# ArturKKK/graphcast-lite

Measured on AMD Instinct MI355X. Metric: training samples/sec (6h windows) + achieved HBM GB/s on mesh GCNConv, higher is better.
Workload: dtype f32

## Files before the change

graphcast-lite_amd/csrc/linear.hip:

```cpp
#include "common.h"
#include "mfma_io.h"
#include "x3.h"

namespace {

using namespace gcl::mfma_io;

#include "gemm_tile.h"

#define gcl_lin_sync() ((abl & 8) != 0)

constexpr int lin_min_waves(int NS, int KT) { return (NS <= 2 && KT <= 64) ? 3 : (NS <= 2 && KT <= 128) ? 2 : 1; }
constexpr bool lin_zpre(int NS, int EPI) { return EPI == 1 && NS >= 4; }

template <int NS, int EPI, int KT, bool VEC>
__global__ __launch_bounds__(256, lin_min_waves(NS, KT)) void linear_mfma_kernel(const float* __restrict__ X, int64_t ldx,
                                                          const float* __restrict__ in_slope,
                                                          const float* __restrict__ W, int32_t ldw, int32_t trans,
                                                          const float* __restrict__ bias, float* __restrict__ Y,
                                                          int64_t ldy, int64_t rows, int32_t K, int32_t N,
                                                          const float* __restrict__ Z, int64_t ldz,
                                                          const float* __restrict__ z_slope,
                                                          double* __restrict__ slope_part, int32_t akind,
                                                          int32_t abl) {
  extern __shared__ __align__(16) float smem[];
  const int KE = (K + 3) & ~3;
  const int KP = KE + 2;
  float* Wl = smem;
  float* Xl = smem + (size_t)NS * 32 * KP;
  const int tid = threadIdx.x, lane = tid & 63, wave = tid >> 6;
  const int NT = blockDim.x;
  const int TM = (NT >> 6) * 32;

  for (int base = 0; base < NS * 32 * KE; base += NT * 8) {
    float wv[8];
#pragma unroll
    for (int u = 0; u < 8; ++u) {
      const int idx = base + u * NT + tid;
      const int j = idx / KE, k = idx - j * KE;
      const bool ok = (idx < NS * 32 * KE) && (j < N) && (k < K);
      const float* src = ok ? (trans ? W + (int64_t)k * ldw + j : W + (int64_t)j * ldw + k)
                            : reinterpret_cast<const float*>(zero4);
      wv[u] = *src;
    }
#pragma unroll
    for (int u = 0; u < 8; ++u) {
      const int idx = base + u * NT + tid;
      const int j = idx / KE, k = idx - j * KE;
      if (idx < NS * 32 * KE) Wl[j * KP + k] = wv[u];
    }
  }
  const float slope = in_slope ? *in_slope : 1.f;
  const bool act = EPI == EPI_BIAS && akind != gcl::kActNone;
  const bool silu = akind == gcl::kActSilu;
  float* Xw = Xl + (size_t)wave * 32 * KP;
  const int64_t ntiles = (rows + TM - 1) / TM;
  double slope_acc = 0.0;
  const float zs = (EPI == EPI_DX && z_slope) ? *z_slope : 1.f;

  constexpr int CPR = VEC ? KT / 4 : KT;
  constexpr int RPI = CPR >= 64 ? 1 : 64 / CPR;
  constexpr int IPR = CPR >= 64 ? CPR / 64 : 1;
  constexpr int NIT = (32 / RPI) * IPR;
  const int rsub = (CPR >= 64) ? 0 : lane / CPR;
  const int csub = (CPR >= 64) ? lane : lane % CPR;
  float pre[VEC ? NIT * 4 : NIT];
  const int64_t rows_ld = (abl & 4) ? 0 : rows;
  auto issue = [&](int64_t tile) {
    const int64_t r0 = tile * TM + wave * 32;
#pragma unroll
    for (int it = 0; it < NIT; ++it) {
      const int64_t row = r0 + (it / IPR) * RPI + rsub;
      const int c = csub + 64 * (it % IPR);
      if (VEC) {
        const bool ok = (c * 4 < K) && (row < rows_ld);
        const float4* p = ok ? reinterpret_cast<const float4*>(X + row * ldx + c * 4) : zero4;
        const float4 v = *p;
        pre[4 * it] = v.x; pre[4 * it + 1] = v.y; pre[4 * it + 2] = v.z; pre[4 * it + 3] = v.w;
      } else {
        const bool ok = (c < K) && (row < rows_ld);
        const float* p = ok ? X + row * ldx + c : reinterpret_cast<const float*>(zero4);
        pre[it] = *p;
      }
    }
  };
  const float pa = (act && !silu) ? slope : 1.f;
  auto commit = [&]() {
    if (act && silu) {
#pragma unroll
      for (int q = 0; q < (VEC ? NIT * 4 : NIT); ++q) pre[q] = gcl::silu_f(pre[q]);
    } else {
#pragma unroll
      for (int q = 0; q < (VEC ? NIT * 4 : NIT); ++q) pre[q] = pre[q] > 0.f ? pre[q] : pre[q] * pa;
    }
#pragma unroll
    for (int it = 0; it < NIT; ++it) {
      const int r = (it / IPR) * RPI + rsub;
      const int c = csub + 64 * (it % IPR);
      if (VEC) {
        if (c * 4 < KE) {
          float2* d = reinterpret_cast<float2*>(Xw + r * KP + c * 4);
          d[0] = make_float2(pre[4 * it], pre[4 * it + 1]);
          d[1] = make_float2(pre[4 * it + 2], pre[4 * it + 3]);
        }
      } else {
        if (c < KE) Xw[r * KP + c] = pre[it];
      }
    }
  };

  float bj[NS];
#pragma unroll
  for (int s = 0; s < NS; ++s) {
    const int j = s * 32 + (lane & 31);
    bj[s] = (EPI == EPI_BIAS && bias && j < N) ? bias[j] : 0.f;
  }
  const bool has_z = (EPI == EPI_DX) && (Z != nullptr);

  issue(blockIdx.x);
  __syncthreads();
  for (int64_t t = blockIdx.x; t < ntiles; t += gridDim.x) {
    if (!gcl_lin_sync()) __builtin_amdgcn_fence(__ATOMIC_ACQ_REL, "wavefront");
    else __syncthreads();
    commit();
    if (gcl_lin_sync()) __syncthreads();
    issue(t + gridDim.x);

    const int64_t r0 = t * TM;
    const int64_t nr = (rows - r0) < TM ? (rows - r0) : TM;
    const __amdgpu_buffer_rsrc_t ry = make_rsrc(Y + r0 * ldy, (abl & 1) ? 0 : win_bytes(nr, ldy, N));
    const __amdgpu_buffer_rsrc_t rz = make_rsrc(has_z ? Z + r0 * ldz : Y, has_z ? win_bytes(nr, ldz, N) : 0);

    f32x16 acc[NS];
#pragma unroll
    for (int s = 0; s < NS; ++s)
#pragma unroll
      for (int r = 0; r < 16; ++r) acc[s][r] = 0.f;

    constexpr bool ZPRE = lin_zpre(NS, EPI);
    float zpre[ZPRE ? NS : 1][16];
    if (ZPRE) {
#pragma unroll
      for (int s = 0; s < NS; ++s) {
        const int j = s * 32 + (lane & 31);
#pragma unroll
        for (int r = 0; r < 16; ++r) {
          const int rr = wave * 32 + d_row(r, lane);
          zpre[ZPRE ? s : 0][r] = buf_ld1(rz, (j < N) ? (unsigned)((rr * ldz + j) * 4) : kOOB);
        }
      }
    }

    const float* ap = Xw + (lane & 31) * KP + 2 * (lane >> 5);
    const float* bp = Wl + (lane & 31) * KP + 2 * (lane >> 5);
    const int nq = (abl & 2) ? 0 : (KE >> 2);
    float2 a_c = *reinterpret_cast<const float2*>(ap);
    float2 b_c[NS];
#pragma unroll
    for (int s = 0; s < NS; ++s) b_c[s] = *reinterpret_cast<const float2*>(bp + s * 32 * KP);
    for (int q = 0; q < nq; ++q) {
      const int qn = (q + 1 < nq) ? q + 1 : q;
      const float2 a_n = *reinterpret_cast<const float2*>(ap + qn * 4);
      float2 b_n[NS];
#pragma unroll
      for (int s = 0; s < NS; ++s) b_n[s] = *reinterpret_cast<const float2*>(bp + s * 32 * KP + qn * 4);
#pragma unroll
      for (int s = 0; s < NS; ++s) acc[s] = __builtin_amdgcn_mfma_f32_32x32x2f32(a_c.x, b_c[s].x, acc[s], 0, 0, 0);
#pragma unroll
      for (int s = 0; s < NS; ++s) acc[s] = __builtin_amdgcn_mfma_f32_32x32x2f32(a_c.y, b_c[s].y, acc[s], 0, 0, 0);
      a_c = a_n;
#pragma unroll
      for (int s = 0; s < NS; ++s) b_c[s] = b_n[s];
    }

#pragma unroll
    for (int s = 0; s < NS; ++s) {
      const int j = s * 32 + (lane & 31);
      const bool jok = j < N;
      if (EPI == EPI_DX) {
        float zv[16];
#pragma unroll
        for (int r = 0; r < 16; ++r) {
          const int rr = wave * 32 + d_row(r, lane);
          if (ZPRE) zv[r] = zpre[ZPRE ? s : 0][r];
          else zv[r] = buf_ld1(rz, jok ? (unsigned)((rr * ldz + j) * 4) : kOOB);
        }
#pragma unroll
        for (int r = 0; r < 16; ++r) {
          const int rr = wave * 32 + d_row(r, lane);
          float v = acc[s][r];
          if (silu) {
            v *= has_z ? gcl::dsilu_f(zv[r]) : 1.f;
          } else {
            const bool neg = has_z && !(zv[r] > 0.f);
            slope_acc += neg ? (double)(v * zv[r]) : 0.0;
            v = neg ? v * zs : v;
          }
          buf_st1<GCL_ST_AUX>(ry, jok ? (unsigned)((rr * ldy + j) * 4) : kOOB, v);
        }
      } else {
#pragma unroll
        for (int r = 0; r < 16; ++r) {
          const int rr = wave * 32 + d_row(r, lane);
          buf_st1<GCL_ST_AUX>(ry, jok ? (unsigned)((rr * ldy + j) * 4) : kOOB, acc[s][r] + bj[s]);
        }
      }
    }
  }

  if (EPI == EPI_DX && slope_part) {
    for (int off = 32; off > 0; off >>= 1) slope_acc += __shfl_down(slope_acc, off, 64);
    __syncthreads();
    double* dred = reinterpret_cast<double*>(smem);
    if (lane == 0) dred[wave] = slope_acc;
    __syncthreads();
    if (tid == 0) {
      double tot = 0.0;
      for (int wv = 0; wv < (NT >> 6); ++wv) tot += dred[wv];
      slope_part[blockIdx.x] = tot;
    }
  }
}

template <int EPI>
__global__ __launch_bounds__(256) void linear_valu_kernel(const float* __restrict__ X, int64_t ldx,
                                                          const float* __restrict__ in_slope,
                                                          const float* __restrict__ W, int32_t ldw, int32_t trans,
                                                          const float* __restrict__ bias, float* __restrict__ Y,
                                                          int64_t ldy, int64_t rows, int32_t K, int32_t N,
                                                          const float* __restrict__ Z, int64_t ldz,
                                                          const float* __restrict__ z_slope,
                                                          double* __restrict__ slope_part, int32_t akind) {
  __shared__ double red[4];
  const float slope = in_slope ? *in_slope : 1.f;
  const bool act = EPI == EPI_BIAS && akind != gcl::kActNone;
  const float zs = (EPI == EPI_DX && z_slope) ? *z_slope : 1.f;
  double slope_acc = 0.0;
  const int64_t total = rows * N;
  for (int64_t idx = (int64_t)blockIdx.x * 256 + threadIdx.x; idx < total; idx += (int64_t)gridDim.x * 256) {
    const int64_t r = idx / N;
    const int j = (int)(idx - r * N);
    float acc = 0.f;
    for (int k = 0; k < K; ++k) {
      float xv = X[r * ldx + k];
      if (act) xv = gcl::act_f(xv, slope, akind);
      const float wv = trans ? W[(int64_t)k * ldw + j] : W[(int64_t)j * ldw + k];
      acc = fmaf(xv, wv, acc);
    }
    if (EPI == EPI_BIAS) {
      if (bias) acc += bias[j];
    } else if (Z) {
      const float z = Z[r * ldz + j];
      if (akind == gcl::kActSilu) {
        acc *= gcl::dsilu_f(z);
      } else if (!(z > 0.f)) {
        slope_acc += (double)(acc * z);
        acc *= zs;
      }
    }
    Y[r * ldy + j] = acc;
  }
  if (EPI == EPI_DX && slope_part) {
    for (int off = 32; off > 0; off >>= 1) slope_acc += __shfl_down(slope_acc, off, 64);
    if ((threadIdx.x & 63) == 0) red[threadIdx.x >> 6] = slope_acc;
    __syncthreads();
    if (threadIdx.x == 0) slope_part[blockIdx.x] = red[0] + red[1] + red[2] + red[3];
  }
}

constexpr int kDwRT = 64;

template <int NO, int NC>
struct DwCfg {
  static constexpr int WO = NO >= 4 ? 4 : NO;
  static constexpr int WC = 4 / WO;
  static constexpr int TO = NO / WO;
  static constexpr int TC = (NC + WC - 1) / WC;
  static constexpr int PRE = 2 * (NO + NC);
  static constexpr int FoutP = NO * 32, FinP = NC * 32;
  static constexpr int min_waves = (PRE <= 8 && TO * TC <= 2) ? 3 : (PRE <= 16 && TO * TC <= 4) ? 2 : 1;
};

template <int NO, int NC, bool VEC>
__global__ __launch_bounds__(256, (DwCfg<NO, NC>::min_waves)) void dw_mfma_kernel(
    const float* __restrict__ dY, int64_t lddy, const float* __restrict__ X, int64_t ldx,
    const float* __restrict__ in_slope, float* __restrict__ part, float* __restrict__ dbpart, int64_t rows,
    int32_t Fin_all, int32_t Fout, int64_t rows_per_block, int32_t akind, int64_t tile_stride) {
  using Cfg = DwCfg<NO, NC>;
  const int ct = blockIdx.y;
  X += (int64_t)ct * 128;
  part += (int64_t)ct * tile_stride;
  if (ct != 0) dbpart = nullptr;
  const int Fin = (Fin_all - ct * 128) < 128 ? (Fin_all - ct * 128) : 128;
  constexpr int WO = Cfg::WO, WC = Cfg::WC, TO = Cfg::TO, TC = Cfg::TC, PRE = Cfg::PRE;
  constexpr int FoutP = Cfg::FoutP, FinP = Cfg::FinP;
  extern __shared__ __align__(16) float smem[];
  float* Yl = smem;
  float* Xl = smem + (size_t)kDwRT * FoutP;
  const int tid = threadIdx.x, lane = tid & 63, wave = tid >> 6;
  const int li = lane & 31, lk = lane >> 5;
  const int wo = wave % WO, wc = wave / WO;
  const float slope = in_slope ? *in_slope : 1.f;
  const bool act = akind != gcl::kActNone;
  const int64_t rb = (int64_t)blockIdx.x * rows_per_block;
  const int64_t re = min(rows, rb + rows_per_block);
  const int nrows = (int)(re - rb);

  f32x16 acc[TO][TC];
#pragma unroll
  for (int a = 0; a < TO; ++a)
#pragma unroll
    for (int c = 0; c < TC; ++c)
#pragma unroll
      for (int r = 0; r < 16; ++r) acc[a][c][r] = 0.f;
  float dbacc[TO];
#pragma unroll
  for (int a = 0; a < TO; ++a) dbacc[a] = 0.f;

  const int rs = tid >> 3, cg = tid & 7;
  float4 pre[PRE];
  const float* ybase = dY + rb * lddy;
  const float* xbase = X + rb * ldx;
  auto ld_slot = [&](const float* base, int rr, int c4, int64_t ld, int F) -> float4 {
    const bool ok = rr < nrows;
    const float* z = reinterpret_cast<const float*>(zero4);
    const float* src = base + (int64_t)rr * ld + c4;
    if (VEC) return *reinterpret_cast<const float4*>((ok && c4 < F) ? src : z);
    float4 v;
    v.x = *((ok && c4 < F) ? src : z);
    v.y = *((ok && c4 + 1 < F) ? src + 1 : z);
    v.z = *((ok && c4 + 2 < F) ? src + 2 : z);
    v.w = *((ok && c4 + 3 < F) ? src + 3 : z);
    return v;
  };
  auto issue = [&](int rel0) {
#pragma unroll
    for (int it = 0; it < PRE; ++it) {
      const int j = it >> 1;
      const int rr = rel0 + rs + 32 * (it & 1);
      if (j < NO) pre[it] = ld_slot(ybase, rr, (cg + 8 * j) * 4, lddy, Fout);
      else pre[it] = ld_slot(xbase, rr, (cg + 8 * (j - NO)) * 4, ldx, Fin);
    }
  };
  auto commit = [&]() {
#pragma unroll
    for (int it = 0; it < PRE; ++it) {
      const int j = it >> 1;
      const int r = rs + 32 * (it & 1);
      float4 v = pre[it];
      if (j < NO) {
        *reinterpret_cast<float4*>(Yl + r * FoutP + (cg + 8 * j) * 4) = v;
      } else {
        if (act) {
          v.x = gcl::act_f(v.x, slope, akind); v.y = gcl::act_f(v.y, slope, akind);
          v.z = gcl::act_f(v.z, slope, akind); v.w = gcl::act_f(v.w, slope, akind);
        }
        *reinterpret_cast<float4*>(Xl + r * FinP + (cg + 8 * (j - NO)) * 4) = v;
      }
    }
  };

  issue(0);
  for (int rel0 = 0; rel0 < nrows; rel0 += kDwRT) {
    __syncthreads();
    commit();
    __syncthreads();
    issue(rel0 + kDwRT);
    const float* yp = Yl + lk * FoutP + li;
    const float* xp = Xl + lk * FinP + li;
    float av[TO], bv[TC];
#pragma unroll
    for (int a = 0; a < TO; ++a) av[a] = yp[(wo + a * WO) * 32];
#pragma unroll
    for (int c = 0; c < TC; ++c) {
      const int sc = wc + c * WC;
      bv[c] = (sc < NC) ? xp[sc * 32] : 0.f;
    }
    for (int k = 0; k < kDwRT; k += 2) {
      const int kn = (k + 2 < kDwRT) ? k + 2 : k;
      float an[TO], bn[TC];
#pragma unroll
      for (int a = 0; a < TO; ++a) an[a] = yp[kn * FoutP + (wo + a * WO) * 32];
#pragma unroll
      for (int c = 0; c < TC; ++c) {
        const int sc = wc + c * WC;
        bn[c] = (sc < NC) ? xp[kn * FinP + sc * 32] : 0.f;
      }
#pragma unroll
      for (int a = 0; a < TO; ++a) {
        dbacc[a] += av[a];
#pragma unroll
        for (int c = 0; c < TC; ++c)
          acc[a][c] = __builtin_amdgcn_mfma_f32_32x32x2f32(av[a], bv[c], acc[a][c], 0, 0, 0);
      }
#pragma unroll
      for (int a = 0; a < TO; ++a) av[a] = an[a];
#pragma unroll
      for (int c = 0; c < TC; ++c) bv[c] = bn[c];
    }
  }

  float* out = part + (size_t)blockIdx.x * FoutP * FinP;
#pragma unroll
  for (int a = 0; a < TO; ++a) {
    const int so = wo + a * WO;
#pragma unroll
    for (int c = 0; c < TC; ++c) {
      const int sc = wc + c * WC;
      if (sc < NC) {
#pragma unroll
        for (int r = 0; r < 16; ++r)
          out[(size_t)(so * 32 + d_row(r, lane)) * FinP + sc * 32 + li] = acc[a][c][r];
      }
    }
    if (dbpart && wc == 0) {
      const float d = dbacc[a] + __shfl_xor(dbacc[a], 32, 64);
      if (lane < 32) dbpart[(size_t)blockIdx.x * FoutP + so * 32 + lane] = d;
    }
  }
}

template <int NO, int NC>
__global__ __launch_bounds__(256, 1) void linear_bwd_fused_kernel(
    const float* __restrict__ dY, int64_t lddy, const float* __restrict__ W, const float* __restrict__ P,
    int64_t ldp, const float* __restrict__ in_slope, float* __restrict__ dX, int64_t lddx, int64_t rows, int32_t Fin,
    int32_t Fout, float* __restrict__ part_dw, float* __restrict__ part_db, float* __restrict__ part_cs,
    double* __restrict__ part_slope) {
  constexpr int FoP = NO * 32, FiP = NC * 32;
  constexpr int KPo = FoP + 2;
  constexpr int TM = 128;
  constexpr int NT = NO * NC;
  constexpr int TPW = (NT + 3) / 4;
  constexpr int CY = FoP / 4;
  constexpr int CP = NC == 3 ? 32 : FiP / 4;
  constexpr int RY = 64 / CY, RP = 64 / CP;
  constexpr int NY = 32 / RY, NP = 32 / RP;
  extern __shared__ __align__(16) float smem[];
  float* Wt = smem;
  float* dYl = Wt + FiP * KPo;
  float* Pl = dYl + TM * KPo;
  const int tid = threadIdx.x, lane = tid & 63, wave = tid >> 6;
  const int li = lane & 31, lk = lane >> 5;

  for (int idx = tid; idx < FiP * FoP; idx += 256) {
    const int c = idx / FoP, o = idx - c * FoP;
    Wt[c * KPo + o] = (c < Fin && o < Fout) ? W[(int64_t)o * Fin + c] : 0.f;
  }
  const bool act = in_slope != nullptr;
  const float slope = act ? *in_slope : 1.f;
  const int64_t ntiles = (rows + TM - 1) / TM;

  f32x16 dw[TPW];
#pragma unroll
  for (int q = 0; q < TPW; ++q)
#pragma unroll
    for (int r = 0; r < 16; ++r) dw[q][r] = 0.f;
  float dbacc[TPW], cs[NC];
#pragma unroll
  for (int q = 0; q < TPW; ++q) dbacc[q] = 0.f;
#pragma unroll
  for (int s2 = 0; s2 < NC; ++s2) cs[s2] = 0.f;
  double slope_acc = 0.0;

  const int ysub = lane / CY, ycol = lane % CY, psub = lane / CP, pcol = lane % CP;
  float4 pre[NY + NP];
  const float4* zero = zero4;
  auto issue = [&](int64_t tile) {
    const int64_t r0 = tile * TM + wave * 32;
#pragma unroll
    for (int it = 0; it < NY; ++it) {
      const int64_t row = r0 + it * RY + ysub;
      const bool ok = (ycol * 4 < Fout) && (row < rows);
      pre[it] = *(ok ? reinterpret_cast<const float4*>(dY + row * lddy + ycol * 4) : zero);
    }
#pragma unroll
    for (int it = 0; it < NP; ++it) {
      const int64_t row = r0 + it * RP + psub;
      const bool ok = (pcol * 4 < Fin) && (row < rows);
      pre[NY + it] = *(ok ? reinterpret_cast<const float4*>(P + row * ldp + pcol * 4) : zero);
    }
  };
  auto commit = [&]() {
#pragma unroll
    for (int it = 0; it < NY; ++it) {
      const int r = wave * 32 + it * RY + ysub;
      float2* d = reinterpret_cast<float2*>(dYl + r * KPo + ycol * 4);
      const float4 v = pre[it];
      d[0] = make_float2(v.x, v.y);
      d[1] = make_float2(v.z, v.w);
    }
#pragma unroll
    for (int it = 0; it < NP; ++it) {
      const int r = wave * 32 + it * RP + psub;
      const float4 v = pre[NY + it];
      if (pcol * 4 < FiP) *reinterpret_cast<float4*>(Pl + r * FiP + pcol * 4) = v;
    }
  };

  issue(blockIdx.x);
  for (int64_t t = blockIdx.x; t < ntiles; t += gridDim.x) {
    __syncthreads();
    commit();
    __syncthreads();
// ... 713 lines not shown
    return gcl::x3_linear_fwd(x, ldx, act, act == GCL_ACT_PRELU ? slope : nullptr, W, bias, y, ldy, rows, Fin, Fout,
                              (hipStream_t)stream);
  if (!addend && ldw == Fin && (use_valu() || panel_fits(Fin, Fout, vec_x, false, (ldw % 4 == 0) && gcl::aligned16(W))))
    return launch_linear<EPI_BIAS>(x, ldx, act == GCL_ACT_PRELU ? slope : nullptr, W, Fin, 0, bias, y, ldy, rows, Fin,
                                   Fout, nullptr, 0, nullptr, nullptr, nullptr, (hipStream_t)stream, act);
  return launch_gemm<EPI_BIAS>(x, ldx, act, act == GCL_ACT_PRELU ? slope : nullptr, W, ldw, 0, bias, y, ldy, rows, Fin,
                               Fout, nullptr, 0, addend, ldadd, nullptr, nullptr, (hipStream_t)stream);
}

extern "C" int gcl_linear_fwd(const float* x, int64_t ldx, const float* in_slope, const float* W, const float* bias,
                              float* y, int64_t ldy, int64_t rows, int32_t Fin, int32_t Fout, gcl_stream_t stream) {
  return gcl_dense_fwd(x, ldx, in_slope ? GCL_ACT_PRELU : GCL_ACT_NONE, in_slope, W, Fin, bias, nullptr, 0, y, ldy, rows,
                       Fin, Fout, stream);
}

static size_t slope_parts_cap(int64_t rows, int32_t Fin) {
  const int64_t g = (int64_t)gt_geom(rows, Fin).grid;
  return (size_t)(g > 4096 ? g : 4096);
}

extern "C" size_t gcl_linear_bwd_ws_bytes(int64_t rows, int32_t Fin, int32_t Fout) {
  size_t nc = (size_t)(Fin + 31) / 32;
  if (nc > 4) nc = 4;
  const size_t FinP = nc * 32;
  size_t no = (size_t)(Fout + 31) / 32;
  no = no <= 2 ? no : no <= 4 ? 4 : 8;
  const size_t FoutP = no * 32;
  const size_t dw = (size_t)kDwBlocks * FoutP * (FinP + 1) * sizeof(float);
  const size_t sl = slope_parts_cap(rows, Fin) * sizeof(double);
  return dw + sl;
}

extern "C" int gcl_dense_bwd_dx(const float* dy, int64_t lddy, const float* W, int64_t ldw, const float* z, int64_t ldz,
                                int32_t act, const float* slope, float* d_slope, const float* addend, int64_t ldadd,
                                float* dx, int64_t lddx, int64_t rows, int32_t Fin, int32_t Fout, void* ws,
                                size_t ws_bytes, gcl_stream_t stream) {
  GCL_CHECK_ARG(dy && W && dx, "dense_bwd_dx: null argument");
  GCL_CHECK_ARG(lddy >= Fout && lddx >= Fin && ldw >= Fin && (!addend || ldadd >= Fin), "dense_bwd_dx: leading dimension too small");
  if (int rc = check_act("dense_bwd_dx", act, slope)) return rc;
  GCL_CHECK_ARG(act == GCL_ACT_NONE || (z && ldz >= Fin), "dense_bwd_dx: activation given without its pre-activation z");
  hipStream_t st = (hipStream_t)stream;
  const float* sl = act == GCL_ACT_PRELU ? slope : nullptr;
  double* slope_part = nullptr;
  if (sl && d_slope) {
    GCL_CHECK_ARG(ws && ws_bytes >= slope_parts_cap(rows, Fin) * sizeof(double) && gcl::aligned16(ws), "dense_bwd_dx: workspace too small");
    slope_part = (double*)ws;
  }
  int nparts = 0, rc;
  const float* zz = act == GCL_ACT_NONE ? nullptr : z;
  const bool vec_x = (Fout % 4 == 0) && (lddy % 4 == 0) && gcl::aligned16(dy);
  if (!addend && ldw == Fin && (use_valu() || panel_fits(Fout, Fin, vec_x, true, (ldw % 4 == 0) && gcl::aligned16(W))))
    rc = launch_linear<EPI_DX>(dy, lddy, nullptr, W, Fin, 1, nullptr, dx, lddx, rows, Fout, Fin, zz, ldz, sl, slope_part,
                               &nparts, st, act);
  else {
    const size_t off = (slope_parts_cap(rows, Fin) * sizeof(double) + 255) & ~(size_t)255;
    const size_t need = off + (size_t)Fin * Fout * sizeof(float);
    if (ws && ws_bytes >= need && gcl::aligned16(ws) && Fout % 4 == 0 && rows >= 4096) {
      float* Wt = reinterpret_cast<float*>(static_cast<char*>(ws) + off);
      hipLaunchKernelGGL(transpose_kernel, dim3((unsigned)gcl::cdiv(Fin, 32), (unsigned)gcl::cdiv(Fout, 32)), dim3(256), 0,
                         st, W, ldw, Wt, Fout, Fin);
      rc = launch_gemm<EPI_DX>(dy, lddy, act, sl, Wt, Fout, 0, nullptr, dx, lddx, rows, Fout, Fin, zz, ldz, addend,
                               ldadd, slope_part, &nparts, st);
    } else {
      rc = launch_gemm<EPI_DX>(dy, lddy, act, sl, W, ldw, 1, nullptr, dx, lddx, rows, Fout, Fin, zz, ldz, addend, ldadd,
                               slope_part, &nparts, st);
    }
  }
  if (rc) return rc;
  if (slope_part && nparts > 0) {
    hipLaunchKernelGGL(reduce_scalar_kernel, dim3(1), dim3(64), 0, st, slope_part, nparts, d_slope);
    GCL_CHECK_LAUNCH();
  }
  return GCL_OK;
}

extern "C" int gcl_linear_bwd_dx(const float* dy, int64_t lddy, const float* W, const float* x, int64_t ldx,
                                 const float* in_slope, float* d_in_slope, float* dx, int64_t lddx, int64_t rows,
                                 int32_t Fin, int32_t Fout, void* ws, size_t ws_bytes, gcl_stream_t stream) {
  GCL_CHECK_ARG(!in_slope || (x && ldx >= Fin), "linear_bwd_dx: in_slope given without the forward input x");
  return gcl_dense_bwd_dx(dy, lddy, W, Fin, in_slope ? x : nullptr, ldx, in_slope ? GCL_ACT_PRELU : GCL_ACT_NONE,
                          in_slope, d_in_slope, nullptr, 0, dx, lddx, rows, Fin, Fout, ws, ws_bytes, stream);
}

static int dw_block(const float* dy, int64_t lddy, const float* x, int64_t ldx, int akind, const float* in_slope,
                    float* dW, int64_t lddw, float* db, int64_t rows, int32_t Fin, int32_t Fout, int32_t accumulate,
                    void* ws, hipStream_t st, gcl_reduce_job* job = nullptr) {
  const int nct = (Fin + 127) / 128;
  const int NC = nct > 1 ? 4 : (Fin + 31) / 32;
  int NO = (Fout + 31) / 32;
  NO = NO <= 2 ? NO : NO <= 4 ? 4 : 8;
  const int FinP = NC * 32, FoutP = NO * 32;
  const size_t lds = (size_t)kDwRT * (FoutP + FinP) * sizeof(float);
  const int64_t cap = (lds > 80 * 1024 ? gcl::kNumCU : kDwBlocks) / nct;
  int64_t nblk = gcl::cdiv(rows, (nct > 1 ? 4 : 2) * kDwRT);
  if (nblk > cap) nblk = cap;
  if (nblk < 1) nblk = 1;
  int64_t rpb = gcl::cdiv(rows, nblk);
  rpb = gcl::cdiv(rpb, kDwRT) * kDwRT;
  nblk = rows > 0 ? gcl::cdiv(rows, rpb) : 1;
  float* part = (float*)ws;
  float* dbpart = part + (size_t)kDwBlocks * FoutP * FinP;
  const int64_t tile_stride = (int64_t)nblk * FoutP * FinP;
  const bool vec = (lddy % 4 == 0) && (ldx % 4 == 0) && gcl::aligned16(dy) && gcl::aligned16(x);
#define GCL_DW3(NO_, NC_, V_)                                                                                     \
  do {                                                                                                            \
    auto kern = dw_mfma_kernel<NO_, NC_, V_>;                                                                     \
    GCL_ENSURE_DYN_LDS(kern, gcl::kLdsBytes);                                                                     \
    hipLaunchKernelGGL(kern, dim3((unsigned)nblk, (unsigned)nct), dim3(256), lds, st, dy, lddy, x, ldx, in_slope, part, \
                       db ? dbpart : nullptr, rows, Fin, Fout, rpb, akind, tile_stride);                          \
  } while (0)
#define GCL_DW2(NO_, NC_)              \
  do {                                 \
    if (vec) GCL_DW3(NO_, NC_, true);  \
    else GCL_DW3(NO_, NC_, false);     \
  } while (0)
#define GCL_DW(NO_)                    \
  do {                                 \
    switch (NC) {                      \
      case 1: GCL_DW2(NO_, 1); break;  \
      case 2: GCL_DW2(NO_, 2); break;  \
      case 3: GCL_DW2(NO_, 3); break;  \
      default: GCL_DW2(NO_, 4); break; \
    }                                  \
  } while (0)
  switch (NO) {
    case 1: GCL_DW(1); break;
    case 2: GCL_DW(2); break;
    case 4: GCL_DW(4); break;
    default: GCL_DW(8); break;
  }
#undef GCL_DW
#undef GCL_DW2
#undef GCL_DW3
  GCL_CHECK_LAUNCH();
  const bool defer = job && nct <= 3 && nblk >= 64 && gcl::aligned16(part) && gcl::aligned16(dbpart) &&
                     tile_stride % 4 == 0 && 2 * tile_stride < ((int64_t)1 << 31);
  if (defer) {
    job[0].part = part;
    job[0].pstride = (int64_t)FoutP * FinP;
    job[0].nparts = (int32_t)nblk;
    for (int c = 0; c < nct; ++c) {
      const int fi = Fin - c * 128 < 128 ? Fin - c * 128 : 128;
      job[0].seg[c].out = dW + c * 128;
      job[0].seg[c].poff = (int32_t)(c * tile_stride);
      job[0].seg[c].count = Fout * FinP;
      job[0].seg[c].pld = FinP;
      job[0].seg[c].cols = fi;
      job[0].seg[c].ldo = (int32_t)lddw;
      job[0].seg[c].acc = accumulate ? 1 : 0;
    }
    if (db) {
      job[1].part = dbpart;
      job[1].pstride = FoutP;
      job[1].nparts = (int32_t)nblk;
      job[1].seg[0].out = db;
      job[1].seg[0].poff = 0;
      job[1].seg[0].count = FoutP;
      job[1].seg[0].pld = FoutP;
      job[1].seg[0].cols = Fout;
      job[1].seg[0].ldo = Fout;
      job[1].seg[0].acc = accumulate ? 1 : 0;
    }
    return GCL_OK;
  }
  for (int ct = 0; ct < nct; ct += 3) {
    RedSeg seg[3] = {{nullptr, 0, 0, 1, 0, 0, 0}, {nullptr, 0, 0, 1, 0, 0, 0}, {nullptr, 0, 0, 1, 0, 0, 0}};
    for (int q = 0; q < 3 && ct + q < nct; ++q) {
      const int c = ct + q;
      const int fi = Fin - c * 128 < 128 ? Fin - c * 128 : 128;
      GCL_CHECK_ARG((int64_t)c * tile_stride < ((int64_t)1 << 31), "dense_bwd_dw: partial workspace offset overflows");
      seg[q] = RedSeg{dW + c * 128, (int32_t)(c * tile_stride), Fout * FinP, FinP, fi, (int32_t)lddw, accumulate};
    }
    launch_reduce_multi(part, (int)nblk, (int64_t)FoutP * FinP, seg[0], seg[1], seg[2], st);
    GCL_CHECK_LAUNCH();
  }
  if (db) return gcl::launch_reduce_parts(dbpart, (int)nblk, (int64_t)FoutP, FoutP, db, Fout, 1, Fout, accumulate, st);
  return GCL_OK;
}

static int dense_bwd_dw_impl(const float* dy, int64_t lddy, const float* x, int64_t ldx, int32_t act,
                             const float* slope, float* dW, int64_t lddw, float* db, int64_t rows, int32_t Fin,
                             int32_t Fout, int32_t accumulate, void* ws, size_t ws_bytes, gcl_stream_t stream,
                             gcl_reduce_job* job) {
  if (job) memset(job, 0, 2 * sizeof(*job));
  if (Fout > 256) job = nullptr;
  GCL_CHECK_ARG(dy && x && dW, "dense_bwd_dw: null argument");
  GCL_CHECK_ARG(lddy >= Fout && ldx >= Fin && lddw >= Fin, "dense_bwd_dw: leading dimension too small");
  GCL_CHECK_ARG(Fin >= 1 && Fout >= 1, "dense_bwd_dw: bad shape");
  GCL_CHECK_ARG(lddw < (1 << 30), "dense_bwd_dw: lddw too large");
  if (int rc = check_act("dense_bwd_dw", act, slope)) return rc;
  GCL_CHECK_ARG(ws && ws_bytes >= gcl_linear_bwd_ws_bytes(rows, Fin, Fout), "dense_bwd_dw: workspace too small");
  const float* sl = act == GCL_ACT_PRELU ? slope : nullptr;
  for (int o0 = 0; o0 < Fout; o0 += 256) {
    const int fo = Fout - o0 < 256 ? Fout - o0 : 256;
    int rc = dw_block(dy + o0, lddy, x, ldx, act, sl, dW + (int64_t)o0 * lddw, lddw, db ? db + o0 : nullptr, rows, Fin,
                      fo, accumulate, ws, (hipStream_t)stream, job);
    if (rc) return rc;
  }
  return GCL_OK;
}

extern "C" int gcl_dense_bwd_dw(const float* dy, int64_t lddy, const float* x, int64_t ldx, int32_t act,
                                const float* slope, float* dW, int64_t lddw, float* db, int64_t rows, int32_t Fin,
                                int32_t Fout, int32_t accumulate, void* ws, size_t ws_bytes, gcl_stream_t stream) {
  return dense_bwd_dw_impl(dy, lddy, x, ldx, act, slope, dW, lddw, db, rows, Fin, Fout, accumulate, ws, ws_bytes, stream,
                           nullptr);
}

extern "C" int gcl_dense_bwd_dw_deferred(const float* dy, int64_t lddy, const float* x, int64_t ldx, int32_t act,
                                         const float* slope, float* dW, int64_t lddw, float* db, int64_t rows,
                                         int32_t Fin, int32_t Fout, int32_t accumulate, void* ws, size_t ws_bytes,
                                         gcl_stream_t stream, gcl_reduce_job* job) {
  GCL_CHECK_ARG(job, "dense_bwd_dw_deferred: null job");
  return dense_bwd_dw_impl(dy, lddy, x, ldx, act, slope, dW, lddw, db, rows, Fin, Fout, accumulate, ws, ws_bytes, stream,
                           job);
}

extern "C" int gcl_linear_bwd_dw_deferred(const float* dy, int64_t lddy, const float* x, int64_t ldx,
                                          const float* in_slope, float* dW, float* db, int64_t rows, int32_t Fin,
                                          int32_t Fout, int32_t accumulate, void* ws, size_t ws_bytes,
                                          gcl_stream_t stream, gcl_reduce_job* job) {
  GCL_CHECK_ARG(job, "linear_bwd_dw_deferred: null job");
  return dense_bwd_dw_impl(dy, lddy, x, ldx, in_slope ? GCL_ACT_PRELU : GCL_ACT_NONE, in_slope, dW, Fin, db, rows, Fin, Fout,
                           accumulate, ws, ws_bytes, stream, job);
}

extern "C" int gcl_linear_bwd_dw(const float* dy, int64_t lddy, const float* x, int64_t ldx, const float* in_slope,
                                 float* dW, float* db, int64_t rows, int32_t Fin, int32_t Fout, int32_t accumulate,
                                 void* ws, size_t ws_bytes, gcl_stream_t stream) {
  return gcl_dense_bwd_dw(dy, lddy, x, ldx, in_slope ? GCL_ACT_PRELU : GCL_ACT_NONE, in_slope, dW, Fin, db, rows, Fin,
                          Fout, accumulate, ws, ws_bytes, stream);
}

static bool fused_ok(const float* dy, int64_t lddy, const float* x, int64_t ldx, const float* dx, int64_t lddx,
                     int32_t Fin, int32_t Fout) {
  const int off = gcl::env_int("GCL_NO_FUSED_BWD", 0) != 0;
  if (off || use_valu()) return false;
  return Fout <= 64 && Fin <= 96 && (lddy >= ((Fout + 3) & ~3)) && (Fin % 4 == 0) && (lddy % 4 == 0) && (ldx % 4 == 0) &&
         (lddx >= Fin) && gcl::aligned16(dy) && gcl::aligned16(x) && dx != nullptr;
}

extern "C" size_t gcl_linear_bwd_all_ws_bytes(int64_t rows, int32_t Fin, int32_t Fout) {
  const size_t FiP = (size_t)((Fin + 31) / 32) * 32, FoP = (size_t)((Fout + 31) / 32) * 32;
  const size_t fused = (size_t)3 * gcl::kNumCU * (FoP * FiP + FoP + FiP) * sizeof(float) + (size_t)3 * gcl::kNumCU * 8 + 64;
  size_t sep = gcl_linear_bwd_ws_bytes(rows, Fin, Fout);
  const size_t cs = gcl_colsum_ws_bytes(rows, Fin);
  if (cs > sep) sep = cs;
  return fused > sep ? fused : sep;
}

static int bwd_all_impl(const float* dy, int64_t lddy, const float* W, const float* x, int64_t ldx,
                        const float* in_slope, float* d_in_slope, float* dx, int64_t lddx, float* dW,
                        float* db, float* colsum_dx, int64_t rows, int32_t Fin, int32_t Fout,
                        int32_t accumulate, void* ws, size_t ws_bytes, gcl_stream_t stream, gcl_reduce_job* job) {
  if (job) memset(job, 0, sizeof(*job));
  GCL_CHECK_ARG(dy && W && x && dx && dW, "linear_bwd_all: null argument");
  GCL_CHECK_ARG(ws && ws_bytes >= gcl_linear_bwd_all_ws_bytes(rows, Fin, Fout), "linear_bwd_all: workspace too small");
  hipStream_t st = (hipStream_t)stream;
  const int acc_dw = (accumulate & GCL_ACC_DW) ? 1 : 0, acc_db = (accumulate & GCL_ACC_DB) ? 1 : 0,
            acc_cs = (accumulate & GCL_ACC_COLSUM) ? 1 : 0;
  if (!fused_ok(dy, lddy, x, ldx, dx, lddx, Fin, Fout) || rows == 0) {
    int rc;
    if (db && acc_db != acc_dw) {
      rc = gcl_linear_bwd_dw(dy, lddy, x, ldx, in_slope, dW, nullptr, rows, Fin, Fout, acc_dw, ws, ws_bytes, stream);
      if (rc) return rc;
      rc = gcl_colsum(dy, lddy, rows, Fout, db, acc_db, ws, ws_bytes, stream);
    } else {
      rc = gcl_linear_bwd_dw(dy, lddy, x, ldx, in_slope, dW, db, rows, Fin, Fout, acc_dw, ws, ws_bytes, stream);
    }
    if (rc) return rc;
    rc = gcl_linear_bwd_dx(dy, lddy, W, in_slope ? x : nullptr, ldx, in_slope, d_in_slope, dx, lddx, rows, Fin, Fout,
                           ws, ws_bytes, stream);
    if (rc) return rc;
    if (colsum_dx) rc = gcl_colsum(dx, lddx, rows, Fin, colsum_dx, acc_cs, ws, ws_bytes, stream);
    return rc;
  }
  const int NO = (Fout + 31) / 32, NC = (Fin + 31) / 32;
  const int FoP = NO * 32, FiP = NC * 32;
  const int no64 = gcl::env_int("GCL_NO_FUSED64", 0) != 0;
  const bool use64 = (NC == 2) && !no64;
  const bool use_x3 = use64 && gcl::x3_linear_bwd_applicable(dy, lddy, x, ldx, dx, lddx, Fin, Fout);
  const int64_t ntiles = gcl::cdiv(rows, use64 ? 64 : 128);
  const int64_t cap = use64 ? 3 * gcl::kNumCU : gcl::kNumCU;
  const int nblk = use_x3 ? gcl::x3_linear_bwd_blocks(rows) : (int)(ntiles < cap ? ntiles : cap);
  const size_t rec_f = (size_t)FoP * FiP + FoP + FiP;
  float* part_dw = (float*)ws;
  float* part_db = part_dw + (size_t)FoP * FiP;
  float* part_cs = part_db + FoP;
  double* part_sl = (double*)(((uintptr_t)(part_dw + (size_t)3 * gcl::kNumCU * rec_f) + 15) & ~(uintptr_t)15);
  const bool want_slope = in_slope && d_in_slope;
  if (use_x3) {
    if (int rc = gcl::x3_linear_bwd(dy, lddy, W, x, ldx, in_slope, dx, lddx, rows, Fin, Fout, part_dw, db ? part_db : nullptr,
                                    colsum_dx ? part_cs : nullptr, want_slope ? part_sl : nullptr, st))
      return rc;
  } else if (use64) {
    const size_t lds64 = ((size_t)FiP * (FoP + 2) + 64 * (size_t)(FoP + 2) + 64 * (size_t)FiP) * sizeof(float);
#define GCL_FB64(NO_)                                                                                             \
  do {                                                                                                            \
    auto kern = linear_bwd_fused64_kernel<NO_>;                                                                   \
    hipLaunchKernelGGL(kern, dim3(nblk), dim3(256), lds64, st, dy, lddy, W, x, ldx, in_slope, dx, lddx, rows, Fin, \
                       Fout, part_dw, db ? part_db : nullptr, colsum_dx ? part_cs : nullptr,                      \
                       want_slope ? part_sl : nullptr);                                                           \
  } while (0)
    if (NO == 1) GCL_FB64(1);
    else GCL_FB64(2);
#undef GCL_FB64
  } else {
  const size_t lds = ((size_t)FiP * (FoP + 2) + 128 * (size_t)(FoP + 2) + 128 * (size_t)FiP) * sizeof(float);
#define GCL_FB(NO_, NC_)                                                                                          \
  do {                                                                                                            \
    auto kern = linear_bwd_fused_kernel<NO_, NC_>;                                                                \
    GCL_ENSURE_DYN_LDS(kern, gcl::kLdsBytes);                                                                     \
    hipLaunchKernelGGL(kern, dim3(nblk), dim3(256), lds, st, dy, lddy, W, x, ldx, in_slope, dx, lddx, rows, Fin,  \
                       Fout, part_dw, db ? part_db : nullptr, colsum_dx ? part_cs : nullptr,                      \
// ... 103 lines not shown
```

graphcast-lite_amd/functional.py:

```python
from typing import List, Optional

import os

import torch

from . import hip


def _grad_slot(p: Optional[torch.Tensor], needs: bool):
    if p is None or not needs:
        return None, False, True
    if p.grad is not None:
        return p.grad, True, True
    return torch.zeros_like(p), False, False


class _Grads:

    def __init__(self, params: List[Optional[torch.Tensor]], needs: List[bool]):
        self.dst, self.acc, self.ret_none = [], [], []
        for p, nd in zip(params, needs):
            d, a, r = _grad_slot(p, nd)
            self.dst.append(d)
            self.acc.append(a)
            self.ret_none.append(r)

    def out(self):
        return tuple(None if r else d for d, r in zip(self.dst, self.ret_none))


_ZERO = {}


def _token(like: torch.Tensor, shape):
    z = _ZERO.get(like.device)
    if z is None:
        if like.is_cuda and torch.cuda.is_current_stream_capturing():
            return like.new_zeros(()).expand(shape)
        with torch.inference_mode(False):
            z = _ZERO[like.device] = torch.zeros((), dtype=torch.float32, device=like.device)
    return z.expand(shape)


_ONE = {}


def const_one(like: torch.Tensor):
    one = _ONE.get(like.device)
    if one is None:
        if like.is_cuda and torch.cuda.is_current_stream_capturing():
            return None
        with torch.inference_mode(False):
            one = _ONE[like.device] = torch.ones((), dtype=torch.float32, device=like.device)
    return one


def _loss_grad_inplace() -> bool:
    return os.environ.get("GCL_NO_LOSS_GRAD_INPLACE", "0") != "1"


def _wide_in_place(dy: torch.Tensor, Fp: int):
    if dy.dim() != 3 or dy.dtype != torch.float32 or not dy.is_cuda:
        return None
    B, rows, Fo = dy.shape
    if Fo > Fp or rows == 0 or dy.stride(2) != 1 or dy.stride(1) != Fp or dy.stride(0) != rows * Fp or dy.data_ptr() % 16:
        return None
    off = dy.storage_offset()
    if (off + B * rows * Fp) * 4 > dy.untyped_storage().nbytes():
        return None
    return torch.as_strided(dy, (B, rows, Fp), (rows * Fp, Fp, 1), off)


def _flat3(x: torch.Tensor):
    if x.dim() == 2:
        x = x.unsqueeze(0)
    if not x.is_contiguous():
        x = x.contiguous()
    return x


class MLPFn(torch.autograd.Function):
    @staticmethod
    def forward(ctx, x, owner, has_ln: bool, eps: float, *params):
        L = (len(params) - (2 if has_ln else 0) + 1) // 3
        shape = x.shape
        x2 = hip.rows2d(x.detach())
        zs = []
        cur, slope = x2, None
        out = stats = None
        for k in range(L):
            if 2 <= L - k <= 3:
                tail = hip.mlp_fwd_chain(cur, [params[3 * j].detach() for j in range(k, L)],
                                         [params[3 * j + 1].detach() for j in range(k, L)],
                                         [params[3 * j + 2].detach() for j in range(k, L - 1)], slope,
                                         ln=(params[-2].detach(), params[-1].detach(), eps) if has_ln else None)
                if tail is not None:
                    zs.extend(tail[0])
                    cur, out, stats = tail[0][-1], tail[1], tail[2]
                    break
            W, b = params[3 * k], params[3 * k + 1]
            z = hip.linear_fwd(cur, W.detach(), b.detach(), slope)
            zs.append(z)
            cur = z
            slope = params[3 * k + 2].detach() if k < L - 1 else None
        if out is None:
            out = cur
            if has_ln:
                out, stats = hip.layernorm_fwd(cur, params[-2].detach(), params[-1].detach(), eps)
        ctx.owner, ctx.has_ln, ctx.L = owner, has_ln, L
        ctx.x2, ctx.zs, ctx.stats = x2, zs, stats
        ctx.params = params
        return out.view(shape[:-1] + (out.shape[-1],))

    @staticmethod
    def backward(ctx, dy):
        params, L = ctx.params, ctx.L
        needs = list(ctx.needs_input_grad[4:])
        G = _Grads(list(params), needs)
        dy2 = hip.rows2d(dy)
        zs = ctx.zs
        if ctx.has_ln:
            gi, bi = len(params) - 2, len(params) - 1
            dgam = G.dst[gi] if G.dst[gi] is not None else torch.zeros_like(params[gi])
            dbet = G.dst[bi] if G.dst[bi] is not None else torch.zeros_like(params[bi])
            dz = hip.layernorm_bwd(dy2, zs[-1], params[gi].detach(), ctx.stats, dgam, dbet, G.acc[gi] and G.acc[bi])
        else:
            dz = dy2
        dx = None
        for k in range(L - 1, -1, -1):
            W = params[3 * k].detach()
            inp = ctx.x2 if k == 0 else zs[k - 1]
            slope = None if k == 0 else params[3 * k - 1].detach()
            wi, bi = 3 * k, 3 * k + 1
            dW = G.dst[wi] if G.dst[wi] is not None else torch.zeros_like(params[wi])
            db = G.dst[bi]
            if k > 0:
                dz = hip.linear_bwd_all(dz, W, inp, slope, G.dst[3 * k - 1], dW, db, None, G.acc[wi], acc_db=G.acc[bi])
            elif ctx.needs_input_grad[0]:
                dx = hip.linear_bwd_all(dz, W, inp, None, None, dW, db, None, G.acc[wi], acc_db=G.acc[bi],
                                        act=hip.ACT_NONE)
            elif db is not None and G.acc[bi] != G.acc[wi]:
                hip.linear_bwd_dw(dz, inp, None, dW, None, G.acc[wi])
                hip.colsum(dz, db, G.acc[bi])
            else:
                hip.linear_bwd_dw(dz, inp, None, dW, db, G.acc[wi])
        if dx is not None:
            dx = dx.view(dy.shape[:-1] + (dx.shape[-1],))
        return (dx, None, None, None) + G.out()


_LN_COLSUM = os.environ.get("GCL_NO_LN_COLSUM", "0") in ("0", "")
_ROWS_OUT = os.environ.get("GCL_NO_ROWS_OUT", "0") in ("0", "")


def _row_skip() -> bool:
    return os.environ.get("GCL_NO_ROW_SKIP", "0") in ("0", "")


def _split_grad() -> bool:
    return os.environ.get("GCL_NO_SPLIT_GRAD", "0") in ("0", "")


def _split_out() -> bool:
    return os.environ.get("GCL_NO_SPLIT_OUT", "0") in ("0", "")


def _compact_store() -> bool:
    return os.environ.get("GCL_NO_COMPACT_STORE", "0") in ("0", "")


def _fold_sum(g3, inv_fold, r: int, B: int, dst):
    if r > 1:
        hip.gather2_rows(g3, inv_fold, None, None, B * r, B, sum_batch=True, out=dst, deal=r)
    elif r == 1:
        tmp = hip.gather2_rows(g3, inv_fold, None, None, B * r, B, sum_batch=True)
        hip.copy_rows(tmp.view(B, r, g3.shape[-1]), dst)


def _lat_first_layer_bwd(lat, enc3, dz3, W, dW, acc_dw: bool, want_dx: bool, Pc=None, enc_shape=None, dzc=None):
    _, _, inv_a, inv_fold = lat.maps
    B, ne, D = enc_shape if enc3 is None else enc3.shape
    G, Md, r = lat.G, lat.Md, lat.r
    nc = Md + r
    Fo = dz3.shape[-1]
    dz3 = dz3 if dz3.is_contiguous() else dz3.contiguous()
    if dzc is None:
        dzc = torch.empty(B, nc, Fo, dtype=torch.float32, device=dz3.device)
        if Md > 0:
            hip.gather2_rows(dz3, inv_a[G: G + Md], None, None, Md, B, out=dzc[:, :Md])
    _fold_sum(dz3, inv_fold, r, B, dzc[:, Md:])
    if Pc is None:
        Pc = hip.copy_rows(enc3[:, G:, :], torch.empty(B, nc, D, dtype=torch.float32, device=dz3.device))
    if not want_dx:
        hip.linear_bwd_dw(dzc.view(B * nc, Fo), Pc.view(B * nc, D), None, dW, None, acc_dw)
        dxc = None
    else:
        dxc = hip.linear_bwd_all(dzc.view(B * nc, Fo), W, Pc.view(B * nc, D), None, None, dW, None, None, acc_dw,
                                 act=hip.ACT_NONE).view(B, nc, D)
    if GradLanding.keep_tail(lat.landing, dxc):
        return None
    buf, _ = GradLanding.tail(lat.landing)
    if dxc is None:
        return None
    out = buf if buf is not None else torch.zeros(B, ne, D, dtype=torch.float32, device=dz3.device)
    hip.copy_rows(dxc, out[:, G:])
    return None if buf is not None else out


class LatSource:

    def __init__(self, tab, maps, M: int, G: int, Md: int, r: int, landing=None, smap=None, tab_c=None, tail=None):
        self.tab, self.maps, self.M, self.G, self.Md, self.r, self.landing = tab, maps, M, G, Md, r, landing
        self.smap, self.tail = smap, tail
        self._compact = {} if tab_c is None else {tab_c[0]: tab_c[1]}

    def compact_tab(self, ne: int):
        t = self._compact.get(ne)
        if t is None:
            tab = self.tab.to(torch.int64)
            f = -tab - 1
            bq = torch.div(f, ne, rounding_mode="floor")
            flat_c = bq * (self.Md + self.r) + (f - bq * ne - self.G)
            t = torch.where(tab >= 0, tab - self.G, -flat_c - 1).to(torch.int32).contiguous()
            self._compact[ne] = t
        return t


class GCNStackFn(torch.autograd.Function):
# ... 746 lines not shown
```

graphcast-lite_amd/hip.py:

```python
import ctypes as C
import os
from typing import Optional

import torch

_HERE = os.path.dirname(os.path.abspath(__file__))
LIB_PATH = os.environ.get("GCL_LIB") or os.path.join(_HERE, "libgcl_hip.so")

GRAPH_GCN, GRAPH_GAT, GRAPH_MEAN = 0, 1, 2

_lib = None

_i32, _i64, _f32, _vp, _sz = C.c_int32, C.c_int64, C.c_float, C.c_void_p, C.c_size_t

_SIGNATURES = {
    "gcl_version": (C.c_int, []),
    "gcl_last_error": (C.c_char_p, []),
    "gcl_graph_count_edges": (C.c_int, [_vp, _i64, _i32, _i32, C.POINTER(_i64)]),
    "gcl_graph_build_host": (C.c_int, [_vp, _i64, _i32, _i32] + [_vp] * 8),
    "gcl_graph_create": (C.c_int, [_vp, _i64, _i32, _i32, C.POINTER(_vp)]),
    "gcl_graph_destroy": (None, [_vp]),
    "gcl_graph_num_nodes": (_i32, [_vp]),
    "gcl_graph_num_edges": (_i64, [_vp]),
    "gcl_graph_max_in_degree": (_i32, [_vp]),
    "gcl_graph_export_edges": (C.c_int, [_vp, _vp]),
    "gcl_graph_eperm_device": (_vp, [_vp]),
    "gcl_graph_halo_info": (C.c_int, [_vp, _i32, _i32, _vp]),
    "gcl_linear_fwd": (C.c_int, [_vp, _i64, _vp, _vp, _vp, _vp, _i64, _i64, _i32, _i32, _vp]),
    "gcl_linear_bwd_dx": (C.c_int, [_vp, _i64, _vp, _vp, _i64, _vp, _vp, _vp, _i64, _i64, _i32, _i32, _vp, _sz, _vp]),
    "gcl_linear_bwd_dw": (C.c_int, [_vp, _i64, _vp, _i64, _vp, _vp, _vp, _i64, _i32, _i32, _i32, _vp, _sz, _vp]),
    "gcl_linear_bwd_ws_bytes": (_sz, [_i64, _i32, _i32]),
    "gcl_linear_bwd_all": (C.c_int, [_vp, _i64, _vp, _vp, _i64, _vp, _vp, _vp, _i64, _vp, _vp, _vp, _i64, _i32, _i32,
                                     _i32, _vp, _sz, _vp]),
    "gcl_linear_bwd_all_deferred": (C.c_int, [_vp, _i64, _vp, _vp, _i64, _vp, _vp, _vp, _i64, _vp, _vp, _vp, _i64, _i32,
                                              _i32, _i32, _vp, _sz, _vp, _vp]),
    "gcl_reduce_jobs": (C.c_int, [_vp, _i32, _vp]),
    "gcl_layernorm_bwd_deferred": (C.c_int, [_vp, _i64, _i64, _vp, _i32, _i32, _vp, _i64, _vp, _vp, _vp, _i64, _vp, _vp, _vp,
                                             _i32, _i64, _i32, _vp, _sz, _vp, _vp]),
    "gcl_colsum_deferred": (C.c_int, [_vp, _i64, _i64, _i32, _vp, _i32, _vp, _sz, _vp, _vp]),
    "gcl_colsum_split_deferred": (C.c_int, [_vp, _i64, _i64, _vp, _i64, _i64, _i32, _i32, _i32, _i32, _vp, _i32, _vp, _sz,
                                            _vp, _vp]),
    "gcl_linear_bwd_dw_deferred": (C.c_int, [_vp, _i64, _vp, _i64, _vp, _vp, _vp, _i64, _i32, _i32, _i32, _vp, _sz, _vp,
                                             _vp]),
    "gcl_dense_bwd_dw_deferred": (C.c_int, [_vp, _i64, _vp, _i64, _i32, _vp, _vp, _i64, _vp, _i64, _i32, _i32, _i32, _vp,
                                            C.c_size_t, _vp, _vp]),
    "gcl_linear_bwd_all_ws_bytes": (_sz, [_i64, _i32, _i32]),
    "gcl_aggregate": (C.c_int, [_vp, _i32, _vp, _i64, _i64, _vp, _vp, _i64, _i64, _i32, _i32, _vp]),
    "gcl_aggregate_present": (C.c_int, [_vp, _i32, _vp, _i64, _i64, _vp, _vp, _vp, _i64, _i64, _i32, _i32, _vp]),
    "gcl_aggregate_compact_ok": (C.c_int, [_vp, _i32, _i64, _i64, _i64, _i64, _i32, _i32]),
    "gcl_aggregate_compact": (C.c_int, [_vp, _i32, _vp, _i64, _i64, _vp, _vp, _i64, _i64, _vp, _i64, _i64, _i32, _i32, _vp]),
    "gcl_aggregate_heavy_launches": (_i64, []),
    "gcl_aggregate_split": (C.c_int, [_vp, _i32, _vp, _i64, _i64, _vp, _i64, _i64, _i32, _vp, _vp, _i64, _i64, _i32, _i32,
                                      _vp]),
    "gcl_aggregate_head": (C.c_int, [_vp, _i32, _vp, _i64, _i64, _i32, _vp, _vp, _i64, _i64, _i32, _i32, _vp]),
    "gcl_gat_fwd": (C.c_int, [_vp, _vp, _i64, _i64, _vp, _vp, _vp, _vp, _vp, _vp, _vp, _i64, _i64, _i32, _i32, _i32, _vp]),
    "gcl_gat_bwd": (C.c_int, [_vp, _vp, _i64, _i64, _vp, _i64, _i64, _vp, _vp, _vp, _vp, _vp, _vp, _i64, _i64,
                              _vp, _vp, _vp, _i32, _i32, _i32, _i32, _vp, _sz, _vp]),
    "gcl_gat_bwd_ws_bytes": (_sz, [_i64, _i32, _i32, _i32, _i32]),
    "gcl_gat_fwd_tab": (C.c_int, [_vp, _vp, _i64, _i64, _vp, _vp, _vp, _vp, _vp, _vp, _vp, _vp, _i64, _i64, _i32, _i32, _i32, _vp]),
    "gcl_gat_bwd_tab": (C.c_int, [_vp, _vp, _i64, _i64, _vp, _i64, _i64, _vp, _vp, _vp, _vp, _vp, _vp, _vp, _i64, _i64,
                                  _vp, _vp, _vp, _i32, _i32, _i32, _i32, _vp, _sz, _vp]),
    "gcl_gat_tab_ok": (C.c_int, [_vp, _i64, _i32, _i32]),
    "gcl_gat_alpha_to_edge_order": (C.c_int, [_vp, _vp, _vp, _i32, _vp]),
    "gcl_gat_prune": (C.c_int, [_vp, _vp, _f32, _vp, C.POINTER(_i64), _vp, _sz, _vp]),
    "gcl_gat_prune_ws_bytes": (_sz, [_i64]),
    "gcl_layernorm_fwd": (C.c_int, [_vp, _i64, _vp, _vp, _f32, _vp, _i64, _vp, _i64, _i32, _vp]),
    "gcl_layernorm_bwd": (C.c_int, [_vp, _i64, _vp, _i64, _vp, _vp, _vp, _i64, _vp, _vp, _i32, _i64, _i32, _vp, _sz, _vp]),
    "gcl_layernorm_bwd_cs": (C.c_int, [_vp, _i64, _vp, _i64, _vp, _vp, _vp, _i64, _vp, _vp, _vp, _i32, _i64, _i32, _vp, _sz, _vp]),
    "gcl_layernorm_bwd_map": (C.c_int, [_vp, _i64, _i64, _vp, _i32, _vp, _i64, _vp, _vp, _vp, _i64, _vp, _vp, _vp, _i32, _i64,
                                        _i32, _vp, _sz, _vp]),
    "gcl_layernorm_fwd_map_skip": (C.c_int, [_vp, _i64, _vp, _vp, _f32, _vp, _i64, _i64, _vp, _i32, _vp, _i32, _vp, _i64, _i32,
                                             _vp]),
    "gcl_layernorm_bwd_map_skip": (C.c_int, [_vp, _i64, _i64, _vp, _i32, _vp, _i64, _vp, _vp, _vp, _i64, _vp, _vp, _vp, _i32,
                                             _i64, _i32, _vp, _sz, _vp]),
    "gcl_layernorm_bwd_ws_bytes": (_sz, [_i64, _i32]),
    "gcl_graphnorm_fwd": (C.c_int, [_vp, _i64, _i64, _vp, _vp, _f32, _vp, _i64, _i64, _vp, _i32, _i32, _i32, _vp, _sz, _vp]),
    "gcl_graphnorm_bwd": (C.c_int, [_vp, _i64, _i64, _vp, _i64, _i64, _vp, _vp, _f32, _vp, _i64, _i64, _vp, _vp,
                                    _i32, _i32, _i32, _i32, _vp, _sz, _vp]),
    "gcl_graphnorm_ws_bytes": (_sz, [_i32, _i32, _i32]),
    "gcl_colsum": (C.c_int, [_vp, _i64, _i64, _i32, _vp, _i32, _vp, _sz, _vp]),
    "gcl_colsum_ws_bytes": (_sz, [_i64, _i32]),
    "gcl_colsum_split": (C.c_int, [_vp, _i64, _i64, _vp, _i64, _i64, _i32, _i32, _i32, _i32, _vp, _i32, _vp, _sz, _vp]),
    "gcl_assemble_input": (C.c_int, [_vp, _vp, _vp, _vp, _i64, _i32, _i32, _i32, _i32, _i32, _vp]),
    "gcl_assemble_input_tail": (C.c_int, [_vp, _vp, _vp, _vp, _i32, _vp, _i64, _i32, _i32, _i32, _i32, _i32, _vp]),
    "gcl_wmse_fwd_bwd": (C.c_int, [_vp, _i64, _i64, _vp, _i64, _i64, _vp, _i64, _i64, _vp, _vp, _f32, _f32, _vp,
                                   _vp, _vp, _vp, _i32, _i32, _i32, _vp, _sz, _vp]),
    "gcl_wmse_fwd_bwd_ld": (C.c_int, [_vp, _i64, _i64, _vp, _i64, _i64, _vp, _i64, _i64, _vp, _vp, _f32, _f32, _vp, _i64, _i64,
                                      _vp, _vp, _vp, _i32, _i32, _i32, _vp, _sz, _vp]),
    "gcl_ar_step_bwd": (C.c_int, [_vp, _vp, _vp, _vp, _i32, _i32, _vp, _vp, _i32, _i32, _i32, _i32, _vp]),
    "gcl_ar_step_bwd_ld": (C.c_int, [_vp, _i64, _i64, _vp, _vp, _vp, _i32, _i32, _vp, _i64, _i64, _vp, _i32, _i32, _i32, _i32,
                                     _vp]),
    "gcl_pad_rows": (C.c_int, [_vp, _i64, _i64, _i32, _i32, _vp, _i64, _i64, _i32, _i32, _i32, _vp]),
    "gcl_zero": (C.c_int, [_vp, _sz, _vp]),
    "gcl_wmse_ws_bytes": (_sz, [_i32, _i32, _i32]),
    "gcl_adam_step": (C.c_int, [_vp, _vp, _vp, _vp, _i64, _f32, _f32, _f32, _f32, _f32, _i32, _f32, _vp]),
    "gcl_adam_step_dev": (C.c_int, [_vp, _vp, _vp, _vp, _i64, _f32, _f32, _f32, _f32, _f32, _vp, _vp, _f32, _vp]),
    "gcl_adam_step_groups": (C.c_int, [_vp, _vp, _vp, _vp, _i64, _vp, _i32, _vp, _vp, _vp, _vp, _f32, _f32, _f32, _f32,
                                       _f32, _vp]),
    "gcl_copy_rows": (C.c_int, [_vp, _i64, _i64, _vp, _i64, _i64, _i32, _i32, _i32, _vp]),
    "gcl_dense_fwd": (C.c_int, [_vp, _i64, _i32, _vp, _vp, _i64, _vp, _vp, _i64, _vp, _i64, _i64, _i32, _i32, _vp]),
    "gcl_mlp_fwd_chain_ok": (C.c_int, [_vp, _i64, _i64, _i32, _i32, _i32] + [_vp, _i64, _i32] * 3 + [_vp, _vp, _i64, _vp]),
    "gcl_mlp_fwd_chain": (C.c_int, [_vp, _i64, _i64, _i32, _i32, _vp, _i32, _vp, _vp, _vp, _i64, _i32]
                          + [_vp, _vp, _vp, _vp, _i64, _i32] * 2 + [_vp, _vp, _f32, _vp, _i64, _vp, _vp]),
    "gcl_dense_bwd_dx": (C.c_int, [_vp, _i64, _vp, _i64, _vp, _i64, _i32, _vp, _vp, _vp, _i64, _vp, _i64, _i64, _i32, _i32,
                                   _vp, C.c_size_t, _vp]),
    "gcl_dense_bwd_dw": (C.c_int, [_vp, _i64, _vp, _i64, _i32, _vp, _vp, _i64, _vp, _i64, _i32, _i32, _i32, _vp,
                                   C.c_size_t, _vp]),
    "gcl_gcn_layer_fwd": (C.c_int, [_vp, _vp, _i64, _i64, _i32, _vp, _vp, _vp, _vp, _i64, _i64, _i32, _i32, _i32, _i32, _vp]),
    "gcl_gcn_layer_fwd_rows": (C.c_int, [_vp, _vp, _i64, _i64, _i32, _vp, _vp, _vp, _vp, _i64, _i64, _i32, _i32, _i32, _i32, _i32, _vp]),
    "gcl_gcn_layer_fwd_split": (C.c_int, [_vp, _vp, _i64, _i64, _i32, _vp, _vp, _vp, _vp, _i64, _i64, _vp, _i64, _i64, _i32, _i32, _i32,
                                          _i32, _i32, _vp]),
    "gcl_gcn_layer_fwd_split_ok": (C.c_int, [_vp, _i64, _i64, _i64, _i64, _i64, _i64, _i32, _i32, _i32, _i32, _i32]),
    "gcl_gcn_layer_fwd_present": (C.c_int, [_vp, _vp, _i64, _i64, _i32, _vp, _vp, _vp, _vp, _i64, _i64, _vp, _i32, _i32, _i32, _i32,
                                            _vp]),
    "gcl_layernorm_fwd_map": (C.c_int, [_vp, _i64, _vp, _vp, _f32, _vp, _i64, _i64, _vp, _i32, _vp, _i64, _i32, _vp]),
    "gcl_gcn_layer_fwd_tab": (C.c_int, [_vp, _vp, _i64, _i64, _i64, _vp, _i32, _vp, _vp, _vp, _vp, _i64, _i64, _i32, _i32, _i32, _i32, _vp]),
    "gcl_gcn_layer_fwd_tab_ok": (C.c_int, [_vp, _i64, _i64, _i64, _i32, _i32, _i32]),
    "gcl_segment_reduce": (C.c_int, [_vp, _i64, _i64, _vp, _vp, _i32, _vp, _i64, _i64, _i32, _i32, _i32, _vp]),
    "gcl_edge_combine": (C.c_int, [_vp, _vp, _vp, _i64, _i64, _vp, _vp, _vp, _i64, _i64, _vp, _vp, _i32, _i64, _i32, _vp]),
    "gcl_act_fwd": (C.c_int, [_vp, _vp, _i64, _i32, _vp, _vp]),
    "gcl_act_bwd": (C.c_int, [_vp, _vp, _vp, _i64, _i32, _vp, _vp, _vp, C.c_size_t, _vp]),
    "gcl_act_bwd_ws_bytes": (C.c_size_t, []),
    "gcl_window_pack": (C.c_int, [_vp, _i64, _i32, _i32, _i32, _vp, _vp, _vp, _i32, _i32, _i32, _vp, _vp, _i32, _vp]),
    "gcl_ar_advance": (C.c_int, [_vp, _vp, _i64, _i64, _vp, _i64, _i64, _vp, _vp, _vp, _i64, _i64, _i32, _i32, _i32, _i32,
                                 _i32, _i32, _vp]),
    "gcl_gather2_rows": (C.c_int, [_vp, _i64, _i64, _vp, _vp, _i64, _i64, _vp, _vp, _i64, _i64, _i32, _i32, _i32, _i32, _vp]),
    "gcl_roi_gather_rows": (C.c_int, [_vp, _i32, _i32] + [_vp, _i64, _i64, _i32] * 3 + [_vp, _i64, _i64, _i32, _i32, _vp]),
    "gcl_roi_compose": (C.c_int, [_vp, _i64, _i64, _vp, _i64, _i64, _vp, _vp, _i64, _i64, _i32, _i32, _i32, _vp]),
    "gcl_segment_wsum": (C.c_int, [_vp, _i64, _i64, _i32, _i32, _vp, _vp, _vp, _vp, _i64, _i64, _vp, _i64, _i64, _i32,
                                   _i32, _i32, _i32, _vp]),
    "gcl_cross_update_fwd": (C.c_int, [_vp, _i64, _i64, _vp, _i64, _i64, _vp, _vp, _vp, _f32, _vp, _vp, _vp, _i32, _i32,
                                       _i32, _vp]),
    "gcl_nudge": (C.c_int, [_vp, _i64, _i64, _vp, _i64, _i64, _vp, _f32, _f32, _i32, _vp, _i64, _i64, _i32, _i32, _i32,
                            _vp]),
    "gcl_nudge_rows": (C.c_int, [_vp, _i64, _i64, _vp, _i64, _i64, _vp, _i32, _vp, _vp, _vp, _vp, _i64, _i64, _i32, _i32,
                                 _i32, _vp]),
    "gcl_oi_max_stations": (C.c_int, []),
    "gcl_oi_station_cov": (C.c_int, [_vp, _vp, _i32, C.c_double, C.c_double, C.c_double, _vp, _vp]),
    "gcl_oi_factor": (C.c_int, [_vp, _i32, _vp]),
    "gcl_oi_solve": (C.c_int, [_vp, _i32, _vp, _vp, _vp, _i32, _vp]),
    "gcl_oi_innovation": (C.c_int, [_vp, _i64, _i64, _vp, _i64, _i64, _vp, _vp, _vp, _i32, _i32, _i32, _vp, _vp]),
    "gcl_oi_analysis": (C.c_int, [_vp, _i64, _i64, _vp, _i64, _i64, _vp, _i32, _vp, _vp, _vp, _vp, _i32, _vp, _vp, _vp,
                                  _vp, _i32, _f32, _f32, _f32, _f32, _i32, _vp]),
    "gcl_oi_analysis_rows": (C.c_int, [_vp, _i64, _i64, _vp, _i64, _i64, _vp, _i32, _vp, _vp, _vp, _vp, _i32, _vp, _vp,
                                       _vp, _vp, _i32, _vp, _vp, _f32, _f32, _i32, _vp]),
    "gcl_verify_colstats_ws_bytes": (_sz, [_i32, _i32, _i32, _i32]),
    "gcl_verify_colstats": (C.c_int, [_vp, _i64, _i64, _i32, _i32] + [_vp, _i64, _i64, _vp] * 4
                            + [_vp, _i32, _i32, _vp, _vp, _sz, _vp]),
    "gcl_verify_accumulate": (C.c_int, [_vp, _vp, _i32, _vp, _vp, _vp]),
    "gcl_regrid_blend": (C.c_int, [_vp, _i32, _i64, _i64, _i32, _vp, _vp, _i32, _i32, _vp, _i64, _i64, _vp, _vp, _i64,
                                   _i64, _vp, _i64, _i64, _i32, _vp]),
    "gcl_taper_blend": (C.c_int, [_vp, _vp, _i64, _i64, _vp, _i64, _i64, _vp, _i64, _i64, _i32, _i32, _i32, _vp]),
    "gcl_mos_forest_eval": (C.c_int, [_vp, _vp, _i32, C.c_double, _vp, _i32, _vp, _vp]),
    "gcl_mos_forest_predict": (C.c_int, [_vp, _vp, _i32, C.c_double, _vp, _i32, _i64, _i64, _i64, _i32] + [_i32] * 5
                               + [_vp, _vp, _i32, _i32, _vp, _vp, _vp, _vp, _i32, _vp]),
    "gcl_mos_idw_apply": (C.c_int, [_vp, _i32, _i64, _i64, _i64, _vp, _i64, _i64, _i64, _i32, _i32, _i32, _i32, _vp,
                                    _vp, _vp, _i32, _vp, _i32, C.c_double, C.c_double, _vp, _i32, _vp]),
    "gcl_mos_idw_sweep_ws_bytes": (_sz, [_i32, _i32, _i32, _i32]),
    "gcl_mos_idw_sweep_max_configs": (C.c_int, []),
    "gcl_mos_idw_sweep": (C.c_int, [_vp, _i32, _i64, _i64, _i64, _vp, _i64, _i64, _i64, _i32, _i32, _i32, _vp, _vp, _vp,
                                    _i32, _vp, _i32, _vp, _vp, _i32, _vp, _i32, _i32, _vp, _vp, _vp, _sz, _i32, _vp]),
    "gcl_mos_table_apply": (C.c_int, [_vp, _i32, _i64, _i64, _i64, _vp, _i64, _i64, _i64, _i32, _i32, _i32, _i32, _vp,
                                      _i32, _i32, _vp]),
    "gcl_mos_fit_ws_bytes": (_sz, [_i32, _i32, _i32, _i32, _i32]),
    "gcl_mos_fit_bin": (C.c_int, [_vp, _i32, _i32, _vp, _vp, _vp, _i64, _vp]),
    "gcl_mos_fit_gradients": (C.c_int, [_vp, _vp, _vp, _i32, _vp]),
    "gcl_mos_fit_histogram": (C.c_int, [_vp, _i64, _i32, _vp, _vp, _i32, _i32, _vp, _vp, _vp, _sz, _vp]),
# ... 648 lines not shown
    _check(lib().gcl_colsum_split(*args, ws.data_ptr(), ws.numel(), _stream()))
    return out


def gat_tab_ok(graph: Graph, H: int, Cc: int) -> bool:
    return bool(lib().gcl_gat_tab_ok(graph.handle, H * Cc, int(H), int(Cc)))


def gat_fwd(graph: Graph, h3, att_src, att_dst, bias, H, Cc, need_alpha=True, tab=None):
    B, n, HC = h3.shape
    if tab is not None:
        n = graph.n
        assert h3.is_contiguous()
    dev = h3.device
    a_s = torch.empty(B, n, H, dtype=torch.float32, device=dev)
    a_d = torch.empty(B, n, H, dtype=torch.float32, device=dev)
    alpha = torch.empty(B, graph.e, H, dtype=torch.float32, device=dev) if need_alpha else None
    y = torch.empty(B, n, Cc, dtype=torch.float32, device=dev)
    tok = _probe_begin("gat_fwd", graph=graph, B=B, H=H, C=Cc, alpha=need_alpha)
    if tab is not None:
        _check(lib().gcl_gat_fwd_tab(graph.handle, _p(h3), h3.stride(1), h3.stride(0), _pi(tab), _p(att_src), _p(att_dst),
                                     _p(bias), _p(a_s), _p(a_d), _p(alpha), _p(y), Cc, n * Cc, B, H, Cc, _stream()))
    else:
        _check(lib().gcl_gat_fwd(graph.handle, _p(h3), h3.stride(1), h3.stride(0), _p(att_src), _p(att_dst), _p(bias),
                                 _p(a_s), _p(a_d), _p(alpha), _p(y), Cc, n * Cc, B, H, Cc, _stream()))
    _probe_end(tok)
    return y, a_s, a_d, alpha


def gat_bwd(graph: Graph, dy3, h3, att_src, att_dst, a_s, a_d, alpha, d_att_src, d_att_dst, d_bias, accumulate, H, Cc, tab=None):
    B, n, HC = h3.shape
    if tab is not None:
        n = graph.n
    dy3 = dy3.contiguous()
    dh = torch.empty(B, n, HC, dtype=torch.float32, device=h3.device)
    nb = lib().gcl_gat_bwd_ws_bytes(graph.e, n, B, H, Cc)
    ws = workspace(nb, h3.device)
    tok = _probe_begin("gat_bwd", graph=graph, B=B, H=H, C=Cc)
    if tab is not None:
        _check(lib().gcl_gat_bwd_tab(graph.handle, _p(dy3), Cc, n * Cc, _p(h3), h3.stride(1), h3.stride(0), _pi(tab), _p(att_src),
                                     _p(att_dst), _p(a_s), _p(a_d), _p(alpha), _p(dh), HC, n * HC, _p(d_att_src),
                                     _p(d_att_dst), _p(d_bias), 1 if accumulate else 0, B, H, Cc, ws.data_ptr(), ws.numel(),
                                     _stream()))
    else:
        _check(lib().gcl_gat_bwd(graph.handle, _p(dy3), Cc, n * Cc, _p(h3), h3.stride(1), h3.stride(0), _p(att_src),
                                 _p(att_dst), _p(a_s), _p(a_d), _p(alpha), _p(dh), HC, n * HC, _p(d_att_src), _p(d_att_dst),
                                 _p(d_bias), 1 if accumulate else 0, B, H, Cc, ws.data_ptr(), ws.numel(), _stream()))
    _probe_end(tok)
    return dh


def gat_alpha_edge_order(graph: Graph, alpha_slots_1sample, H):
    out = torch.empty(graph.e, H, dtype=torch.float32, device=alpha_slots_1sample.device)
    _check(lib().gcl_gat_alpha_to_edge_order(graph.handle, _p(alpha_slots_1sample.contiguous()), _p(out), H, _stream()))
    return out


def gat_prune(graph: Graph, alpha_edges, threshold: float) -> torch.Tensor:
    buf = torch.empty(2 * graph.e, dtype=torch.int64)
    kept = _i64(0)
    nb = lib().gcl_gat_prune_ws_bytes(graph.e)
    ws = workspace(nb, alpha_edges.device)
    _check(lib().gcl_gat_prune(graph.handle, _p(alpha_edges.contiguous()), float(threshold), buf.data_ptr(),
                               C.byref(kept), ws.data_ptr(), ws.numel(), _stream()))
    k = kept.value
    return buf[: 2 * k].view(2, k).clone()


def assemble_input(x3, grid_static, mesh_static, tail3=None):
    B, G, Cdyn = x3.shape
    M, Cs = mesh_static.shape
    x3 = x3.contiguous()
    out = torch.empty(B, G + M, Cdyn + Cs, dtype=torch.float32, device=x3.device)
    if tail3 is not None and tail3.is_contiguous() and tail3.shape[2] == Cdyn + Cs:
        _check(lib().gcl_assemble_input_tail(_p(x3), _p(grid_static), _p(mesh_static), _p(tail3), tail3.shape[1], _p(out),
                                             Cdyn + Cs, B, G, M, Cdyn, Cs, _stream()))
        return out
    _check(lib().gcl_assemble_input(_p(x3), _p(grid_static), _p(mesh_static), _p(out), Cdyn + Cs, B, G, M, Cdyn, Cs, _stream()))
    if tail3 is not None:
        copy_rows(tail3, out[:, G + M - tail3.shape[1]:, :])
    return out


def wmse_fwd_bwd(delta3, x_last3, y3, node_w, chan_w, inv_wsum, grad_scale, want_grad=True, want_state=False,
                 loss_prev=None, ldd_out=None):
    B, G, Cc = delta3.shape
    dev = delta3.device
    if delta3.stride(2) != 1:
        delta3 = delta3.contiguous()
    dd = None
    if want_grad:
        dd = torch.empty(B, G, ldd_out if ldd_out else Cc, dtype=torch.float32, device=dev)
    st = torch.empty(B, G, Cc, dtype=torch.float32, device=dev) if want_state else None
    loss = torch.empty((), dtype=torch.float32, device=dev)
    nb = lib().gcl_wmse_ws_bytes(B, G, Cc)
    ws = workspace(nb, dev)
    xl = x_last3
    head = (_p(delta3), delta3.stride(1), delta3.stride(0), _p(xl), xl.stride(1) if xl is not None else 0,
            xl.stride(0) if xl is not None else 0, _p(y3), y3.stride(1), y3.stride(0), _p(node_w), _p(chan_w), float(inv_wsum),
            float(grad_scale), _p(dd))
    tail = (_p(st), _p(loss_prev), _p(loss), B, G, Cc, ws.data_ptr(), ws.numel(), _stream())
    if ldd_out:
        assert ldd_out >= Cc
        _check(lib().gcl_wmse_fwd_bwd_ld(*head, int(ldd_out), G * int(ldd_out), *tail))
        return loss, (dd[..., :Cc] if dd is not None else None), st
    _check(lib().gcl_wmse_fwd_bwd(*head, *tail))
    return loss, dd, st


def adam_step(p, g, m, v, lr, beta1, beta2, eps, weight_decay, step, grad_scale=1.0):
    _check(lib().gcl_adam_step(_p(p), _p(g), _p(m), _p(v), p.numel(), lr, beta1, beta2, eps, weight_decay, int(step),
                               float(grad_scale), _stream()))


def adam_step_dev(p, g, m, v, lr, beta1, beta2, eps, weight_decay, step_dev, bc_dev, grad_scale=1.0):
    assert step_dev.dtype == torch.int32 and step_dev.is_cuda
    _check(lib().gcl_adam_step_dev(_p(p), _p(g), _p(m), _p(v), p.numel(), lr, beta1, beta2, eps, weight_decay,
                                   step_dev.data_ptr(), _p(bc_dev), float(grad_scale), _stream()))


def adam_step_groups(p, g, m, v, chunk_param, active, lr, step, bc, beta1, beta2, eps, weight_decay, grad_scale=1.0):
    P = step.numel()
    assert p.is_cuda and p.numel() % 64 == 0 and chunk_param.numel() == p.numel() // 64
    assert step.dtype == active.dtype == chunk_param.dtype == torch.int32 and lr.dtype == bc.dtype == torch.float32
    assert active.numel() == lr.numel() == P and bc.numel() == 2 * P
    _check(lib().gcl_adam_step_groups(_p(p), _p(g), _p(m), _p(v), p.numel(), _pi(chunk_param), P, _pi(active),
                                      _p(lr), _pi(step), _p(bc), beta1, beta2, eps, weight_decay, float(grad_scale),
                                      _stream()))


def copy_rows(src3, dst3):
    B, rows, F = src3.shape
    _check(lib().gcl_copy_rows(_p(src3), src3.stride(1), src3.stride(0), _p(dst3), dst3.stride(1), dst3.stride(0), B, rows, F, _stream()))
    return dst3


def _pi(t):
    if t is None:
        return None
    assert t.is_cuda and t.dtype == torch.int32 and t.is_contiguous()
    return t.data_ptr()


def gather2_rows(a3, map_a, b3, map_b, nd: int, B: int, sum_batch: bool = False, out=None, deal: int = 0):
    F = a3.shape[-1]
    if sum_batch and deal > 1:
        assert out is not None and nd % deal == 0 and out.shape == (nd // deal, deal, F) and out.stride(2) == 1
        flag = deal
    else:
        if out is None:
            out = torch.empty(1 if sum_batch else B, nd, F, dtype=torch.float32, device=a3.device)
        assert out.shape == (1 if sum_batch else B, nd, F) and out.stride(2) == 1
        flag = 1 if sum_batch else 0
    bsa = a3.stride(0) if (a3.shape[0] > 1 or sum_batch) else 0
    bsb = 0 if b3 is None else (b3.stride(0) if b3.shape[0] > 1 else 0)
    _check(lib().gcl_gather2_rows(_p(a3), a3.stride(1), bsa, _pi(map_a), _p(b3), 0 if b3 is None else b3.stride(1),
                                  bsb, _pi(map_b), _p(out), out.stride(1), out.stride(0), B, nd, F, flag, _stream()))
    return out


def roi_gather_rows(rows, rows_src: int, srcs, Fp: int, B: int, out=None):
    n = rows.numel() if rows is not None else out.shape[1]
    if out is None:
        out = torch.empty(B, n, Fp, dtype=torch.float32, device=srcs[0].device)
    assert out.shape == (B, n, Fp) and out.stride(2) == 1 and len(srcs) <= 3
    args = []
# ... 1248 lines not shown
```

graphcast-lite_amd/models.py:

```python
import contextlib
import math
import os
import sys
from collections import OrderedDict
from typing import Optional, Tuple

import numpy as np
import torch
import torch.nn as nn

from . import hip
from .config import (
    DataConfig,
    GraphBlock,
    GraphBuildingConfig,
    GraphLayerType,
    MLPBlock,
    ModelConfig,
    PipelineConfig,
)
from .create_graphs import (create_decoding_graph, create_encoding_graph, create_processing_graph,
                            create_product_graph)
from .functional import (AssembleFn, EdgeLayout, GATLayerFn, Gather2Fn, GCNStackFn, GradLanding, GraphNormFn, InteractionNetFn,
                         LatSource, LayerNormFn, MeanAggFn, MeshLatFn, MLPFn)
# ... 592 lines not shown
        c.mi = mi
        self._compact = c
        return c

    _fold_invariant_rows = os.environ.get("GCL_NO_FOLD", "0") in ("0", "")

    def _fold_setup(self, c, B: int, device):
        G, M, Md, Mi = self._num_grid_nodes, self._num_mesh_nodes, c.Md, c.Mi
        r = -(-Mi // B)
        ne = G + Md + r
        Cs, Cdyn = self.init_mesh_features.shape[1], self._dyn_size
        f = type("Fold", (), {})()
        f.r, f.ne = r, ne
        stat = self.init_mesh_features.to(device)
        f.mstat = torch.cat([c.mstat_dep.to(device), torch.zeros(r, Cs, device=device)], dim=0).contiguous()
        x_fold = torch.zeros(B * r, Cdyn + Cs, device=device)
        x_fold[:Mi, Cdyn:] = stat[c.mi.to(device)]
        f.x_fold = x_fold.view(B, r, Cdyn + Cs)
        i32 = lambda t: t.to(torch.int32).contiguous().to(device)
        j = torch.arange(Mi)
        map_b = torch.full((M,), -1, dtype=torch.int64)
        map_b[c.mi] = (j // r) * ne + G + Md + (j % r)
        inv_fold = torch.full((B * r,), -1, dtype=torch.int64)
        inv_fold[:Mi] = c.mi
        if c.perm is not None:
            map_b = map_b[c.perm[0]]
            inv_fold[:Mi] = c.perm[1][c.mi]
        f.maps = (c.maps_mesh[0], i32(map_b), c.maps_mesh[2], i32(inv_fold))
        dep = c.maps_mesh[2].cpu().to(torch.int64)[G: G + Md]
        f.smap = None
        if Md > 0 and int(dep.min()) >= 0 and int(dep.max()) < M and torch.unique(dep).numel() == Md:
            smap = torch.full((M,), -1, dtype=torch.int64)
            smap[dep] = torch.arange(Md)
            f.smap = i32(smap)
        f.tab = torch.where(f.maps[0] >= 0, f.maps[0], -f.maps[1] - 1).to(torch.int32).contiguous()
        f.tab_c = (ne, LatSource(f.tab, f.maps, M, G, Md, r).compact_tab(ne))
        rd = -(-Md // B) if Md > 0 else 0
        f.rd, f.nm = rd, G + r + rd
        x_dep = torch.zeros(B * rd, Cdyn + Cs, device=device)
        x_dep[:Md, Cdyn:] = c.mstat_dep.to(device)
        f.x_tail2 = torch.cat([f.x_fold, x_dep.view(B, rd, Cdyn + Cs)], dim=1).contiguous()
        f.mstat2 = torch.zeros(r + rd, Cs, device=device)
        ea = torch.full((ne,), -1, dtype=torch.int64)
        ea[:G] = torch.arange(G)
        ea[G + Md:] = G + torch.arange(r)
        eb = torch.full((ne,), -1, dtype=torch.int64)
        d = torch.arange(Md)
        if rd > 0:
            eb[G: G + Md] = (d // rd) * f.nm + G + r + (d % rd)
        einv_a = torch.full((G + r,), -1, dtype=torch.int64)
        einv_a[:G] = torch.arange(G)
        einv_a[G:] = G + Md + torch.arange(r)
        einv_f = torch.full((B * rd,), -1, dtype=torch.int64)
        einv_f[:Md] = G + d
        f.maps_e = (i32(ea), i32(eb), i32(einv_a), i32(einv_f))
        dinv_a = torch.cat([c.maps_dec[2], torch.full((r,), -1, dtype=torch.int32, device=device)]).contiguous()
        f.maps_dec = (c.maps_dec[0], c.maps_dec[1], dinv_a, c.maps_dec[3])
        f.dec_head_identity = bool(torch.equal(dinv_a[:G].cpu().to(torch.int64), torch.arange(G)))
        c.fold[B] = f
        return f

    def _forward_compact(self, X: torch.Tensor, attention_threshold=0.0, _landing=False, _latents_discarded=False, **kwargs):
        G, M = self._num_grid_nodes, self._num_mesh_nodes
        squeeze = X.dim() == 2 or (X.dim() == 3 and X.shape[0] == 1)
        X3 = X if X.dim() == 3 else X.unsqueeze(0)
        B = X3.shape[0]
        if self.use_product_graph:
            X3 = self._product_stage(X3)
        c = getattr(self, "_compact", None) or self._compact_setup(X3.device)
        if self._fold_invariant_rows:
            f = c.fold.get(B) or self._fold_setup(c, B, X3.device)
            land = GradLanding(G, head_identity=f.dec_head_identity) if _landing and self._grad_landing else None
            lat_pre = None
            ekw = {"_split": land} if (land is not None and self.encoder.graph_layer.layer_type == GraphLayerType.ConvGCN) else {}
            D_enc = self._encoder_width() if ekw else None
            if D_enc is not None and self._decoder_input_channel(land, _latents_discarded, squeeze):
                land.open_decoder_input(B, G + c.U, D_enc, X3.device, f.maps_dec[3], f.maps_dec[1][G:])
                ln = self.processor.graph_layer._final_ln()
                if ln is not None and ln.mode == "node" and ln.in_channels == D_enc:
                    lat_pre = self._lat_source(c, f, torch.empty(B, c.Md + f.r, D_enc, device="meta"), land)
                    if lat_pre is not None:
                        land.want_split_out()
            if self._mlp_on_folded_rows and self.encoder.mlp is not None and f.rd > 0:
                x_m = AssembleFn.apply(X3, self.init_grid_features, f.mstat2, f.x_tail2)
                h_m = self.encoder.mlp(X=x_m)
                x_g = MeshLatFn.apply(h_m, f.maps_e, f.ne, G + f.r, f.rd, None)
                enc_c = self.encoder.graph_layer(X=x_g, edge_index=c.enc_graph, **ekw)
            else:
                x_c = AssembleFn.apply(X3, self.init_grid_features, f.mstat, f.x_fold if f.r > 0 else None)
                enc_c = self.encoder.forward(X=x_c, edge_index=c.enc_graph, **ekw)
            tail = land.split_tail() if land is not None else None
            if tail is not None:
                lat_src, lat_pre.tail = lat_pre, tail
            else:
                lat_src = self._lat_source(c, f, enc_c, land)
            if lat_src is None:
                mesh_lat = MeshLatFn.apply(enc_c, f.maps, M, G + c.Md, f.r, land)
            maps_dec = f.maps_dec
        else:
            land = None
            lat_src = None
            maps_dec = c.maps_dec
            x_c = AssembleFn.apply(X3, self.init_grid_features, c.mstat_dep)
            enc_c = self.encoder.forward(X=x_c, edge_index=c.enc_graph)
            inv = self.encoder.forward(X=c.x_inv, edge_index=c.empty_graph) if c.Mi > 0 else None
            mesh_lat = Gather2Fn.apply(enc_c, inv, c.maps_mesh, M, B)
        if land is not None and land.dec_buf is None and self._decoder_input_channel(land, _latents_discarded, squeeze):
            land.open_decoder_input(B, G + c.U, enc_c.shape[-1], enc_c.device, maps_dec[3], maps_dec[1][G:])
        if self.using_sparse_gat:
            pg = self._processing_graph_tiled() if c.perm is not None else self.processing_graph
            processed, new_edge_index = self.processor.forward(
                X=mesh_lat, edge_index=pg, attention_threshold=attention_threshold, _land=land, **kwargs)
            self.processing_graph = self._processing_graph_from_tiled(new_edge_index) if c.perm is not None else new_edge_index
        elif self.using_interaction_net:
            processed = self.processor.forward(X=mesh_lat, edge_index=self.processing_graph,
                                               attention_threshold=attention_threshold,
                                               edge_attr=self._processing_edge_features)
        else:
            pg = self._processing_graph_tiled() if c.perm is not None else self.processing_graph
            processed = self.processor.forward(X=enc_c if lat_src is not None else mesh_lat, edge_index=pg,
                                               attention_threshold=attention_threshold, _lat=lat_src, _land=land)
        dec_in = Gather2Fn.apply(enc_c, processed, maps_dec, G + c.U, B, land)
        gcn_dec = self.decoder.graph_layer.layer_type == GraphLayerType.ConvGCN
        decoded = self.decoder.forward(X=dec_in, edge_index=c.dec_graph, **({"_out_rows": G} if gcn_dec else {}))
        out, grid_lat = (decoded if gcn_dec else decoded[:, :G, :]), enc_c[:, :G, :]
        if c.perm is not None and not _landing:
            pos_dev = getattr(c, "perm_pos_dev", None)
            if pos_dev is None or pos_dev.device != processed.device:
                pos_dev = c.perm_pos_dev = c.perm[1].to(processed.device)
            processed = processed.index_select(1, pos_dev)
        if squeeze:
            return out[0], grid_lat[0], processed[0]
        return out, grid_lat, processed

    _lat_through_table = os.environ.get("GCL_NO_LAT_TABLE", "0") in ("0", "")
    _mlp_on_folded_rows = os.environ.get("GCL_NO_MLP_FOLD", "0") in ("0", "")
    _ln_into_decoder_input = os.environ.get("GCL_NO_LN_MAP", "0") in ("0", "")

    def _decoder_input_channel(self, land, latents_discarded: bool, squeeze: bool) -> bool:
        return (land is not None and self._ln_into_decoder_input and latents_discarded and not squeeze
                and self.processor.graph_layer.layer_type in (GraphLayerType.ConvGCN, GraphLayerType.GATConv,
                                                              GraphLayerType.SparseGATConv))

    def _encoder_width(self):
        gl = self.encoder.graph_layer
        convs = [m for m in gl.layers if isinstance(m, GCNConv)]
        if gl.layer_type != GraphLayerType.ConvGCN or not convs or gl._final_ln() is not None:
            return None
        return int(convs[-1].lin.weight.shape[0])

    def _lat_source(self, c, f, enc_c, land):
        if not self._lat_through_table or c.perm is None or self.processor.mlp is not None:
            return None
        gl = self.processor.graph_layer
        if gl.layer_type == GraphLayerType.GATConv:
            first = gl.layers[0]
            if not isinstance(first, GATConv) or first.heads != 1 or enc_c.dim() != 3 or first.lin.weight.shape[1] != enc_c.shape[-1]:
                return None
            g = _graphs.get(self._processing_graph_tiled(), self._num_mesh_nodes, hip.GRAPH_GAT)
            if not hip.gat_tab_ok(g, 1, first.lin.weight.shape[0]):
                return None
            return LatSource(f.tab, f.maps, self._num_mesh_nodes, self._num_grid_nodes, c.Md, f.r, land, smap=f.smap,
                             tab_c=f.tab_c)
        if gl.layer_type != GraphLayerType.ConvGCN:
            return None
        convs = [m for m in gl.layers if isinstance(m, GCNConv)]
        if not convs or enc_c.dim() != 3 or convs[0].lin.weight.shape[1] != enc_c.shape[-1]:
            return None
        g = _graphs.get(self._processing_graph_tiled(), self._num_mesh_nodes, hip.GRAPH_GCN)
        if not hip.gcn_layer_tab_ok(g, enc_c, convs[0].lin.weight.shape[0]):
            return None
        return LatSource(f.tab, f.maps, self._num_mesh_nodes, self._num_grid_nodes, c.Md, f.r, land, smap=f.smap,
                         tab_c=f.tab_c)

    def forward_with_latents(self, X: torch.Tensor, attention_threshold=0.0, _landing=False, _latents_discarded=False,
                             **kwargs):
        if self._compact_eligible():
            return self._forward_compact(X, attention_threshold, _landing, _latents_discarded, **kwargs)
        G = self._num_grid_nodes
        if X.dim() == 3 and X.shape[0] == 1:
            X = X.squeeze(0)
        if self.use_product_graph:
            X = self._product_stage(X)
        X = self._preprocess_input(grid_node_features=X)
        encoded = self.encoder.forward(X=X, edge_index=self.encoding_graph)
        grid_node_features = encoded[..., :G, :]
        mesh_node_features = encoded[..., G:, :]
        if self.using_sparse_gat:
            processed, new_edge_index = self.processor.forward(
                X=mesh_node_features, edge_index=self.processing_graph, attention_threshold=attention_threshold,
                **kwargs)
            self.processing_graph = new_edge_index
        elif self.using_interaction_net:
            processed = self.processor.forward(
                X=mesh_node_features, edge_index=self.processing_graph, attention_threshold=attention_threshold,
                edge_attr=self._processing_edge_features)
        else:
            processed = self.processor.forward(
                X=mesh_node_features, edge_index=self.processing_graph, attention_threshold=attention_threshold)
        processed_features = torch.cat((grid_node_features, processed), dim=-2)
        if self.decoder.graph_layer.layer_type == GraphLayerType.ConvGCN:
            decoded = self.decoder.forward(X=processed_features, edge_index=self.decoding_graph, _out_rows=G)
            return decoded, grid_node_features, processed
        decoded = self.decoder.forward(X=processed_features, edge_index=self.decoding_graph)
        return decoded[..., :G, :], grid_node_features, processed

    _grad_landing = os.environ.get("GCL_NO_LANDING", "0") in ("0", "")

    def forward(self, X: torch.Tensor, attention_threshold=0.0, **kwargs):
        return self.forward_with_latents(X, attention_threshold, _landing=True, _latents_discarded=True, **kwargs)[0]
```

include/gcl.h:

```cpp
#ifndef GCL_H
#define GCL_H

#include <stddef.h>
#include <stdint.h>

#ifdef __cplusplus
extern "C" {
#endif

#define GCL_VERSION 100

#define GCL_OK 0
#define GCL_EINVAL (-1)
#define GCL_EHIP (-2)
#define GCL_ENOMEM (-3)
#define GCL_EUNSUPPORTED (-4)

typedef struct gcl_graph gcl_graph_t;
typedef void* gcl_stream_t;

int gcl_version(void);
const char* gcl_last_error(void);

#define GCL_GRAPH_GCN 0
// ... 116 lines not shown
int gcl_aggregate_compact(const gcl_graph_t* g, int32_t transpose, const float* h, int64_t ldh, int64_t bsh,
                          const int32_t* smap , float* y, int64_t ldy, int64_t bsy, float* yc, int64_t ldc,
                          int64_t bsc, int32_t B, int32_t F, gcl_stream_t stream);

int gcl_gat_fwd(const gcl_graph_t* g, const float* h, int64_t ldh, int64_t bsh,
                const float* att_src , const float* att_dst , const float* bias ,
                float* a_src , float* a_dst , float* alpha ,
                float* y, int64_t ldy, int64_t bsy, int32_t B, int32_t H, int32_t C,
                gcl_stream_t stream);
int gcl_gat_bwd(const gcl_graph_t* g, const float* dy, int64_t lddy, int64_t bsdy,
                const float* h, int64_t ldh, int64_t bsh, const float* att_src, const float* att_dst,
                const float* a_src, const float* a_dst, const float* alpha,
                float* dh, int64_t lddh, int64_t bsdh, float* d_att_src, float* d_att_dst,
                float* d_bias, int32_t accumulate, int32_t B, int32_t H, int32_t C,
                void* ws, size_t ws_bytes, gcl_stream_t stream);
size_t gcl_gat_bwd_ws_bytes(int64_t e_prime, int32_t n, int32_t B, int32_t H, int32_t C);
int gcl_gat_fwd_tab(const gcl_graph_t* g, const float* h, int64_t ldh, int64_t bsh, const int32_t* tab ,
                    const float* att_src, const float* att_dst, const float* bias, float* a_src, float* a_dst,
                    float* alpha, float* y, int64_t ldy, int64_t bsy, int32_t B, int32_t H, int32_t C,
                    gcl_stream_t stream);
int gcl_gat_bwd_tab(const gcl_graph_t* g, const float* dy, int64_t lddy, int64_t bsdy, const float* h, int64_t ldh,
                    int64_t bsh, const int32_t* tab , const float* att_src, const float* att_dst,
                    const float* a_src, const float* a_dst, const float* alpha, float* dh, int64_t lddh, int64_t bsdh,
                    float* d_att_src, float* d_att_dst, float* d_bias, int32_t accumulate, int32_t B, int32_t H,
                    int32_t C, void* ws, size_t ws_bytes, gcl_stream_t stream);
int gcl_gat_tab_ok(const gcl_graph_t* g, int64_t ldh, int32_t H, int32_t C);
int gcl_gat_alpha_to_edge_order(const gcl_graph_t* g, const float* alpha_slots, float* alpha_edges,
                                int32_t H, gcl_stream_t stream);
int gcl_gat_prune(const gcl_graph_t* g, const float* alpha_edges, float threshold,
                  int64_t* edge_index_out, int64_t* kept, void* ws, size_t ws_bytes,
                  gcl_stream_t stream);
size_t gcl_gat_prune_ws_bytes(int64_t e_prime);

int gcl_layernorm_fwd(const float* x, int64_t ldx, const float* gamma, const float* beta, float eps,
                      float* y, int64_t ldy, float* stats, int64_t rows, int32_t F,
                      gcl_stream_t stream);
int gcl_layernorm_fwd_map(const float* x, int64_t ldx, const float* gamma, const float* beta, float eps, float* y,
                          int64_t ldy, int64_t bsy, const int32_t* pos , int32_t n_per, float* stats,
                          int64_t rows, int32_t F, gcl_stream_t stream);
int gcl_layernorm_bwd(const float* dy, int64_t lddy, const float* x, int64_t ldx, const float* gamma,
                      const float* stats, float* dx, int64_t lddx, float* dgamma, float* dbeta,
                      int32_t accumulate, int64_t rows, int32_t F, void* ws, size_t ws_bytes,
                      gcl_stream_t stream);
int gcl_layernorm_bwd_cs(const float* dy, int64_t lddy, const float* x, int64_t ldx, const float* gamma,
                         const float* stats, float* dx, int64_t lddx, float* dgamma, float* dbeta,
                         float* colsum_dx, int32_t accumulate, int64_t rows, int32_t F, void* ws,
                         size_t ws_bytes, gcl_stream_t stream);
int gcl_layernorm_bwd_map(const float* dy, int64_t lddy, int64_t bsdy, const int32_t* pos, int32_t n_per,
                          const float* x, int64_t ldx, const float* gamma, const float* stats, float* dx,
                          int64_t lddx, float* dgamma, float* dbeta, float* colsum_dx, int32_t accumulate,
                          int64_t rows, int32_t F, void* ws, size_t ws_bytes, gcl_stream_t stream);
int gcl_layernorm_fwd_map_skip(const float* x, int64_t ldx, const float* gamma, const float* beta, float eps, float* y,
                               int64_t ldy, int64_t bsy, const int32_t* pos , int32_t n_per,
                               const int32_t* rlist , int32_t n_list, float* stats, int64_t rows, int32_t F,
                               gcl_stream_t stream);
int gcl_layernorm_bwd_map_skip(const float* dy, int64_t lddy, int64_t bsdy, const int32_t* pos, int32_t n_per,
                               const float* x, int64_t ldx, const float* gamma, const float* stats, float* dx,
                               int64_t lddx, float* dgamma, float* dbeta, float* colsum_dx, int32_t accumulate,
                               int64_t rows, int32_t F, void* ws, size_t ws_bytes, gcl_stream_t stream);
size_t gcl_layernorm_bwd_ws_bytes(int64_t rows, int32_t F);
int gcl_graphnorm_fwd(const float* x, int64_t ldx, int64_t bsx, const float* gamma, const float* beta,
                      float eps, float* y, int64_t ldy, int64_t bsy, float* stats, int32_t B,
                      int32_t n, int32_t F, void* ws, size_t ws_bytes, gcl_stream_t stream);
int gcl_graphnorm_bwd(const float* dy, int64_t lddy, int64_t bsdy, const float* x, int64_t ldx,
                      int64_t bsx, const float* gamma, const float* stats, float eps, float* dx,
                      int64_t lddx, int64_t bsdx, float* dgamma, float* dbeta, int32_t accumulate,
                      int32_t B, int32_t n, int32_t F, void* ws, size_t ws_bytes, gcl_stream_t stream);
size_t gcl_graphnorm_ws_bytes(int32_t B, int32_t n, int32_t F);

int gcl_colsum(const float* x, int64_t ldx, int64_t rows, int32_t F, float* out, int32_t accumulate,
               void* ws, size_t ws_bytes, gcl_stream_t stream);
size_t gcl_colsum_ws_bytes(int64_t rows, int32_t F);
int gcl_colsum_split(const float* a, int64_t lda, int64_t bsa, const float* b, int64_t ldb, int64_t bsb, int32_t head,
                     int32_t n, int32_t B, int32_t F, float* out, int32_t accumulate, void* ws, size_t ws_bytes,
                     gcl_stream_t stream);

int gcl_assemble_input(const float* x , const float* grid_static ,
                       const float* mesh_static , float* out, int64_t ldo, int32_t B,
                       int32_t G, int32_t M, int32_t Cdyn, int32_t Cs, gcl_stream_t stream);
int gcl_assemble_input_tail(const float* x, const float* grid_static, const float* mesh_static, const float* tail,
                            int32_t r, float* out, int64_t ldo, int32_t B, int32_t G, int32_t M, int32_t Cdyn,
                            int32_t Cs, gcl_stream_t stream);

int gcl_wmse_fwd_bwd(const float* delta, int64_t ldd, int64_t bsd, const float* x_last, int64_t ldx,
                     int64_t bsx, const float* y, int64_t ldy_, int64_t bsy, const float* node_w,
                     const float* chan_w, float inv_wsum, float grad_scale, float* d_delta,
                     float* out_state, const float* loss_prev, float* loss_out, int32_t B, int32_t G,
                     int32_t C, void* ws, size_t ws_bytes, gcl_stream_t stream);
int gcl_wmse_fwd_bwd_ld(const float* delta, int64_t ldd, int64_t bsd, const float* x_last, int64_t ldx,
                        int64_t bsx, const float* y, int64_t ldy_, int64_t bsy, const float* node_w,
                        const float* chan_w, float inv_wsum, float grad_scale, float* d_delta, int64_t ldd_out,
                        int64_t bsd_out, float* out_state, const float* loss_prev, float* loss_out, int32_t B,
                        int32_t G, int32_t C, void* ws, size_t ws_bytes, gcl_stream_t stream);
size_t gcl_wmse_ws_bytes(int32_t B, int32_t G, int32_t C);

int gcl_adam_step(float* p, const float* g, float* m, float* v, int64_t count, float lr, float beta1,
                  float beta2, float eps, float weight_decay, int32_t step, float grad_scale,
                  gcl_stream_t stream);

int gcl_adam_step_dev(float* p, const float* g, float* m, float* v, int64_t count, float lr, float beta1,
                      float beta2, float eps, float weight_decay, int32_t* step_dev, float* bc_dev,
                      float grad_scale, gcl_stream_t stream);

int gcl_adam_step_groups(float* p, const float* g, float* m, float* v, int64_t count, const int32_t* chunk_param,
                         int32_t num_params, const int32_t* active, const float* lr, int32_t* step, float* bc,
                         float beta1, float beta2, float eps, float weight_decay, float grad_scale,
                         gcl_stream_t stream);

int gcl_copy_rows(const float* src, int64_t lds, int64_t bss, float* dst, int64_t ldd, int64_t bsd,
                  int32_t B, int32_t rows, int32_t F, gcl_stream_t stream);

int gcl_gcn_layer_fwd(const gcl_graph_t* g, const float* x, int64_t ldx, int64_t bsx, int32_t act,
                      const float* slope, const float* W , const float* bias, float* y,
                      int64_t ldy, int64_t bsy, int32_t B, int32_t Fin, int32_t Fout, int32_t Fout_store,
                      gcl_stream_t stream);
int gcl_gcn_layer_fwd_rows(const gcl_graph_t* g, const float* x, int64_t ldx, int64_t bsx, int32_t act,
                           const float* slope, const float* W , const float* bias, float* y,
                           int64_t ldy, int64_t bsy, int32_t B, int32_t Fin, int32_t Fout, int32_t Fout_store,
                           int32_t rows_out, gcl_stream_t stream);
int gcl_gcn_layer_fwd_split(const gcl_graph_t* g, const float* x, int64_t ldx, int64_t bsx, int32_t act,
                            const float* slope, const float* W , const float* bias, float* ya, int64_t lda,
                            int64_t bsa, float* yb, int64_t ldb, int64_t bsb, int32_t head, int32_t B, int32_t Fin,
                            int32_t Fout, int32_t Fout_store, gcl_stream_t stream);
int gcl_gcn_layer_fwd_split_ok(const gcl_graph_t* g, int64_t ldx, int64_t bsx, int64_t lda, int64_t bsa, int64_t ldb,
                               int64_t bsb, int32_t head, int32_t B, int32_t Fin, int32_t Fout, int32_t Fout_store);
int gcl_gcn_layer_fwd_present(const gcl_graph_t* g, const float* x, int64_t ldx, int64_t bsx, int32_t act,
                              const float* slope, const float* W, const float* bias, float* y, int64_t ldy, int64_t bsy,
                              const int32_t* present , int32_t B, int32_t Fin, int32_t Fout, int32_t Fout_store,
                              gcl_stream_t stream);
int gcl_gcn_layer_fwd_tab(const gcl_graph_t* g, const float* x, int64_t ldx, int64_t bsx, int64_t x_rows,
                          const int32_t* tab , int32_t act, const float* slope, const float* W ,
                          const float* bias, float* y, int64_t ldy, int64_t bsy, int32_t B, int32_t Fin, int32_t Fout,
                          int32_t Fout_store, gcl_stream_t stream);
int gcl_gcn_layer_fwd_tab_ok(const gcl_graph_t* g, int64_t ldx, int64_t bsx, int64_t x_rows, int32_t B, int32_t Fin,
                             int32_t Fout);

int gcl_segment_reduce(const float* src, int64_t ld_src, int64_t bs_src, const int32_t* perm,
                       const int32_t* rowptr , int32_t mean, float* out, int64_t ld_out,
                       int64_t bs_out, int32_t B, int32_t n, int32_t D, gcl_stream_t stream);
int gcl_edge_combine(const float* base, const float* extra, const float* A, int64_t lda, int64_t bsa,
                     const int32_t* ia, const float* sa, const float* C, int64_t ldc, int64_t bsc,
                     const int32_t* ic, float* out, int32_t B, int64_t E, int32_t D,
                     gcl_stream_t stream);
int gcl_act_fwd(const float* x, float* y, int64_t count, int32_t act, const float* slope,
                gcl_stream_t stream);
int gcl_act_bwd(const float* x, const float* dy, float* dx, int64_t count, int32_t act,
                const float* slope, float* d_slope, void* ws, size_t ws_bytes, gcl_stream_t stream);
size_t gcl_act_bwd_ws_bytes(void);

int gcl_window_pack(const uint16_t* series , int64_t T, int32_t n_lon, int32_t n_lat,
                    int32_t Ct, const int64_t* t0, const float* mean, const float* stdv, int32_t C,
                    int32_t obs, int32_t pred, float* X , float* Y ,
                    int32_t B, gcl_stream_t stream);

int gcl_ar_advance(const float* state, const float* delta, int64_t ldd, int64_t bsd, const float* y_step,
                   int64_t ldy, int64_t bsy, const int32_t* chan_kind, float* new_state, float* out,
                   int64_t ldo, int64_t bso, int32_t out_off, int32_t B, int32_t G, int32_t obs, int32_t C,
                   int32_t residual, gcl_stream_t stream);
int gcl_ar_step_bwd(const float* dd, const float* g_loss, const float* g_new, const int32_t* chan_kind,
                    int32_t has_y, int32_t residual, float* d_delta, float* d_state, int32_t B, int32_t G,
                    int32_t obs, int32_t C, gcl_stream_t stream);
int gcl_ar_step_bwd_ld(const float* dd, int64_t ldd, int64_t bsd, const float* g_loss, const float* g_new,
                       const int32_t* chan_kind, int32_t has_y, int32_t residual, float* d_delta, int64_t ldd_out,
                       int64_t bsd_out, float* d_state, int32_t B, int32_t G, int32_t obs, int32_t C,
                       gcl_stream_t stream);

// ... 266 lines not shown
```

Measured before the change: 28300.

## Fuse encoder input assembly into first MLP linear via gathered row sources

Adds a row-source abstraction so the encoder MLP's first linear layer (forward and weight-gradient) reads dynamic, static grid/mesh and tail features directly from their separate tensors instead of materialising an assembled input matrix. This removes the assemble kernel and the write and re-read of the concatenated input through HBM. In exchange, the per-row gather logic is more complex, loads are scattered across several base pointers, and the path only applies when the inputs do not require grad and shapes validate.

```diff
diff --git a/graphcast-lite_amd/csrc/dw_mfma_kernel.inc b/graphcast-lite_amd/csrc/dw_mfma_kernel.inc
--- /dev/null
+++ b/graphcast-lite_amd/csrc/dw_mfma_kernel.inc
@@ -0,0 +1,167 @@
+template <int NO, int NC, bool VEC>
+__global__ __launch_bounds__(256, (DwCfg<NO, NC>::min_waves)) void GCL_KERNEL_NAME(
+    const float* __restrict__ dY, int64_t lddy, const float* __restrict__ X, int64_t ldx,
+    const float* __restrict__ in_slope, float* __restrict__ part, float* __restrict__ dbpart, int64_t rows,
+    int32_t Fin_all, int32_t Fout, int64_t rows_per_block, int32_t akind, int64_t tile_stride GCL_SRC_PARAM) {
+  constexpr bool PARTS = GCL_SRC_PARTS;
+  GCL_SRC_LOCAL
+  using Cfg = DwCfg<NO, NC>;
+  const int ct = blockIdx.y;
+  X += (int64_t)ct * 128;
+  part += (int64_t)ct * tile_stride;
+  if (ct != 0) dbpart = nullptr;
+  const int Fin = (Fin_all - ct * 128) < 128 ? (Fin_all - ct * 128) : 128;
+  constexpr int WO = Cfg::WO, WC = Cfg::WC, TO = Cfg::TO, TC = Cfg::TC, PRE = Cfg::PRE;
+  constexpr int FoutP = Cfg::FoutP, FinP = Cfg::FinP;
+  extern __shared__ __align__(16) float smem[];
+  float* Yl = smem;
+  float* Xl = smem + (size_t)kDwRT * FoutP;
+  const int tid = threadIdx.x, lane = tid & 63, wave = tid >> 6;
+  const int li = lane & 31, lk = lane >> 5;
+  const int wo = wave % WO, wc = wave / WO;
+  const float slope = in_slope ? *in_slope : 1.f;
+  const bool act = akind != gcl::kActNone;
+  const int64_t rb = (int64_t)blockIdx.x * rows_per_block;
+  const int64_t re = min(rows, rb + rows_per_block);
+  const int nrows = (int)(re - rb);
+
+  f32x16 acc[TO][TC];
+#pragma unroll
+  for (int a = 0; a < TO; ++a)
+#pragma unroll
+    for (int c = 0; c < TC; ++c)
+#pragma unroll
+      for (int r = 0; r < 16; ++r) acc[a][c][r] = 0.f;
+  float dbacc[TO];
+#pragma unroll
+  for (int a = 0; a < TO; ++a) dbacc[a] = 0.f;
+
+  const int rs = tid >> 3, cg = tid & 7;
+  float4 pre[PRE];
+  const float* ybase = dY + rb * lddy;
+  const float* xbase = X + rb * ldx;
+  auto ld_slot = [&](const float* base, int rr, int c4, int64_t ld, int F) -> float4 {
+    const bool ok = rr < nrows;
+    const float* z = reinterpret_cast<const float*>(zero4);
+    const float* src = base + (int64_t)rr * ld + c4;
+    if (VEC) return *reinterpret_cast<const float4*>((ok && c4 < F) ? src : z);
+    float4 v;
+    v.x = *((ok && c4 < F) ? src : z);
+    v.y = *((ok && c4 + 1 < F) ? src + 1 : z);
+    v.z = *((ok && c4 + 2 < F) ? src + 2 : z);
+    v.w = *((ok && c4 + 3 < F) ? src + 3 : z);
+    return v;
+  };
+  RowRef xr[2];
+  RowSrc::Walk wk[2];
+  RowSrc::Step st64;
+  if constexpr (PARTS) {
+    st64 = src.step(kDwRT);
+    wk[0] = src.start((uint32_t)(rb + rs));
+    wk[1] = src.start((uint32_t)(rb + rs + 32));
+  }
+  auto locate = [&](int rel0) {
+    if constexpr (PARTS) {
+#pragma unroll
+      for (int h = 0; h < 2; ++h) {
+        xr[h] = src.ref(wk[h], rel0 + rs + 32 * h < nrows);
+        src.advance(wk[h], st64);
+      }
+    }
+  };
+  auto issue = [&](int rel0) {
+#pragma unroll
+    for (int it = 0; it < PRE; ++it) {
+      const int j = it >> 1;
+      const int rr = rel0 + rs + 32 * (it & 1);
+      if (j < NO) {
+        pre[it] = ld_slot(ybase, rr, (cg + 8 * j) * 4, lddy, Fout);
+      } else if constexpr (PARTS) {
+        const int c4 = (cg + 8 * (j - NO)) * 4;
+        const float2 lo = src.piece(xr[it & 1], c4), hi = src.piece(xr[it & 1], c4 + 2);
+        pre[it] = make_float4(lo.x, lo.y, hi.x, hi.y);
+      } else {
+        pre[it] = ld_slot(xbase, rr, (cg + 8 * (j - NO)) * 4, ldx, Fin);
+      }
+    }
+  };
+  auto commit = [&]() {
+#pragma unroll
+    for (int it = 0; it < PRE; ++it) {
+      const int j = it >> 1;
+      const int r = rs + 32 * (it & 1);
+      float4 v = pre[it];
+      if (j < NO) {
+        *reinterpret_cast<float4*>(Yl + r * FoutP + (cg + 8 * j) * 4) = v;
+      } else {
+        if (act) {
+          v.x = gcl::act_f(v.x, slope, akind); v.y = gcl::act_f(v.y, slope, akind);
+          v.z = gcl::act_f(v.z, slope, akind); v.w = gcl::act_f(v.w, slope, akind);
+        }
+        *reinterpret_cast<float4*>(Xl + r * FinP + (cg + 8 * (j - NO)) * 4) = v;
+      }
+    }
+  };
+
+  locate(0);
+  issue(0);
+  locate(kDwRT);
+  for (int rel0 = 0; rel0 < nrows; rel0 += kDwRT) {
+    __syncthreads();
+    commit();
+    __syncthreads();
+    issue(rel0 + kDwRT);
+    locate(rel0 + 2 * kDwRT);
+    const float* yp = Yl + lk * FoutP + li;
+    const float* xp = Xl + lk * FinP + li;
+    float av[TO], bv[TC];
+#pragma unroll
+    for (int a = 0; a < TO; ++a) av[a] = yp[(wo + a * WO) * 32];
+#pragma unroll
+    for (int c = 0; c < TC; ++c) {
+      const int sc = wc + c * WC;
+      bv[c] = (sc < NC) ? xp[sc * 32] : 0.f;
+    }
+    for (int k = 0; k < kDwRT; k += 2) {
+      const int kn = (k + 2 < kDwRT) ? k + 2 : k;
+      float an[TO], bn[TC];
+#pragma unroll
+      for (int a = 0; a < TO; ++a) an[a] = yp[kn * FoutP + (wo + a * WO) * 32];
+#pragma unroll
+      for (int c = 0; c < TC; ++c) {
+        const int sc = wc + c * WC;
+        bn[c] = (sc < NC) ? xp[kn * FinP + sc * 32] : 0.f;
+      }
+#pragma unroll
+      for (int a = 0; a < TO; ++a) {
+        dbacc[a] += av[a];
+#pragma unroll
+        for (int c = 0; c < TC; ++c)
+          acc[a][c] = __builtin_amdgcn_mfma_f32_32x32x2f32(av[a], bv[c], acc[a][c], 0, 0, 0);
+      }
+#pragma unroll
+      for (int a = 0; a < TO; ++a) av[a] = an[a];
+#pragma unroll
+      for (int c = 0; c < TC; ++c) bv[c] = bn[c];
+    }
+  }
+
+  float* out = part + (size_t)blockIdx.x * FoutP * FinP;
+#pragma unroll
+  for (int a = 0; a < TO; ++a) {
+    const int so = wo + a * WO;
+#pragma unroll
+    for (int c = 0; c < TC; ++c) {
+      const int sc = wc + c * WC;
+      if (sc < NC) {
+#pragma unroll
+        for (int r = 0; r < 16; ++r)
+          out[(size_t)(so * 32 + d_row(r, lane)) * FinP + sc * 32 + li] = acc[a][c][r];
+      }
+    }
+    if (dbpart && wc == 0) {
+      const float d = dbacc[a] + __shfl_xor(dbacc[a], 32, 64);
+      if (lane < 32) dbpart[(size_t)blockIdx.x * FoutP + so * 32 + lane] = d;
+    }
+  }
+}
diff --git a/graphcast-lite_amd/csrc/linear.hip b/graphcast-lite_amd/csrc/linear.hip
--- a/graphcast-lite_amd/csrc/linear.hip
+++ b/graphcast-lite_amd/csrc/linear.hip
@@ -10,217 +10,103 @@
 
 #define gcl_lin_sync() ((abl & 8) != 0)
 
+static __device__ float zero_row[128];
+
+__device__ __forceinline__ float2 ldg2(const float* p) {
+  typedef float f32x2 __attribute__((ext_vector_type(2)));
+  const f32x2 v = *reinterpret_cast<const __attribute__((address_space(1))) f32x2*>(reinterpret_cast<uintptr_t>(p));
+  return make_float2(v.x, v.y);
+}
+
+struct RowRef {
+  const float* dyn;
+  const float* st;
+};
+struct RowSrc {
+  const float* x;
+  const float* gs;
+  const float* ms;
+  const float* tail;
+  int32_t G, GM, Cdyn, Cs, r;
+  __device__ __forceinline__ RowRef row(uint32_t b, uint32_t i, bool ok) const {
+    const bool grid = i < (uint32_t)G, tl = i >= (uint32_t)(GM - r);
+    const int64_t toff = ((int64_t)b * r + ((int64_t)i - (GM - r))) * (Cdyn + Cs);
+    const int64_t doff = tl ? toff : ((int64_t)b * G + i) * Cdyn;
+    const int64_t soff = tl ? toff + Cdyn : (int64_t)(grid ? i : i - (uint32_t)G) * Cs;
+    const float* dbase = tl ? tail : x;
+    const float* sbase = tl ? tail : grid ? gs : ms;
+    RowRef rr;
+    rr.dyn = (ok && (tl || grid)) ? dbase + doff : zero_row;
+    rr.st = ok ? sbase + soff : zero_row;
+    return rr;
+  }
+  struct Walk {
+    uint32_t i, xoff, toff, soff;
+  };
+  struct Step {
+    uint32_t rm, dx[2], dt[2], ds[2];
+  };
+  __device__ __forceinline__ Walk start(uint32_t row) const {
+    const uint32_t b = row / (uint32_t)GM, i = row - b * (uint32_t)GM;
+    return Walk{i, (row - b * (uint32_t)(GM - G)) * Cdyn, (row - (b + 1) * (uint32_t)(GM - r)) * (Cdyn + Cs), i * Cs};
+  }
+  __device__ __forceinline__ Step step(uint32_t n) const {
+    const uint32_t q = n / (uint32_t)GM, M = GM - G, T = GM - r, K = Cdyn + Cs;
+    Step s;
+    s.rm = n - q * GM;
+    s.dx[0] = (n - q * M) * Cdyn; s.dx[1] = s.dx[0] - M * Cdyn;
+    s.dt[0] = (n - q * T) * K; s.dt[1] = s.dt[0] - T * K;
+    s.ds[0] = s.rm * Cs; s.ds[1] = s.ds[0] - (uint32_t)GM * Cs;
+    return s;
+  }
+  __device__ __forceinline__ void advance(Walk& w, const Step& s) const {
+    w.i += s.rm;
+    const bool wrap = w.i >= (uint32_t)GM;
+    w.i -= wrap ? (uint32_t)GM : 0u;
+    w.xoff += wrap ? s.dx[1] : s.dx[0];
+    w.toff += wrap ? s.dt[1] : s.dt[0];
+    w.soff += wrap ? s.ds[1] : s.ds[0];
+  }
+  __device__ __forceinline__ RowRef ref(const Walk& w, bool ok) const {
+    const bool grid = w.i < (uint32_t)G, tl = w.i >= (uint32_t)(GM - r);
+    const float* dbase = tl ? tail : x;
+    const float* sbase = tl ? tail : grid ? gs : ms;
+    const uint32_t doff = tl ? w.toff : w.xoff;
+    const uint32_t soff = tl ? w.toff + Cdyn : grid ? w.soff : w.soff - (uint32_t)G * Cs;
+    RowRef rr;
+    rr.dyn = (ok && (tl || grid)) ? dbase + doff : zero_row;
+    rr.st = ok ? sbase + soff : zero_row;
+    return rr;
+  }
+  __device__ __forceinline__ float2 piece(const RowRef& rr, int c) const {
+    const bool d = c < Cdyn;
+    const float* base = d ? rr.dyn : rr.st;
+    const int off = d ? c : c - Cdyn;
+    return ldg2(c < Cdyn + Cs ? base + off : zero_row);
+  }
+};
+
 constexpr int lin_min_waves(int NS, int KT) { return (NS <= 2 && KT <= 64) ? 3 : (NS <= 2 && KT <= 128) ? 2 : 1; }
 constexpr bool lin_zpre(int NS, int EPI) { return EPI == 1 && NS >= 4; }
 
-template <int NS, int EPI, int KT, bool VEC>
-__global__ __launch_bounds__(256, lin_min_waves(NS, KT)) void linear_mfma_kernel(const float* __restrict__ X, int64_t ldx,
-                                                          const float* __restrict__ in_slope,
-                                                          const float* __restrict__ W, int32_t ldw, int32_t trans,
-                                                          const float* __restrict__ bias, float* __restrict__ Y,
-                                                          int64_t ldy, int64_t rows, int32_t K, int32_t N,
-                                                          const float* __restrict__ Z, int64_t ldz,
-                                                          const float* __restrict__ z_slope,
-                                                          double* __restrict__ slope_part, int32_t akind,
-                                                          int32_t abl) {
-  extern __shared__ __align__(16) float smem[];
-  const int KE = (K + 3) & ~3;
-  const int KP = KE + 2;
-  float* Wl = smem;
-  float* Xl = smem + (size_t)NS * 32 * KP;
-  const int tid = threadIdx.x, lane = tid & 63, wave = tid >> 6;
-  const int NT = blockDim.x;
-  const int TM = (NT >> 6) * 32;
-
-  for (int base = 0; base < NS * 32 * KE; base += NT * 8) {
-    float wv[8];
-#pragma unroll
-    for (int u = 0; u < 8; ++u) {
-      const int idx = base + u * NT + tid;
-      const int j = idx / KE, k = idx - j * KE;
-      const bool ok = (idx < NS * 32 * KE) && (j < N) && (k < K);
-      const float* src = ok ? (trans ? W + (int64_t)k * ldw + j : W + (int64_t)j * ldw + k)
-                            : reinterpret_cast<const float*>(zero4);
-      wv[u] = *src;
-    }
-#pragma unroll
-    for (int u = 0; u < 8; ++u) {
-      const int idx = base + u * NT + tid;
-      const int j = idx / KE, k = idx - j * KE;
-      if (idx < NS * 32 * KE) Wl[j * KP + k] = wv[u];
-    }
-  }
-  const float slope = in_slope ? *in_slope : 1.f;
-  const bool act = EPI == EPI_BIAS && akind != gcl::kActNone;
-  const bool silu = akind == gcl::kActSilu;
-  float* Xw = Xl + (size_t)wave * 32 * KP;
-  const int64_t ntiles = (rows + TM - 1) / TM;
-  double slope_acc = 0.0;
-  const float zs = (EPI == EPI_DX && z_slope) ? *z_slope : 1.f;
-
-  constexpr int CPR = VEC ? KT / 4 : KT;
-  constexpr int RPI = CPR >= 64 ? 1 : 64 / CPR;
-  constexpr int IPR = CPR >= 64 ? CPR / 64 : 1;
-  constexpr int NIT = (32 / RPI) * IPR;
-  const int rsub = (CPR >= 64) ? 0 : lane / CPR;
-  const int csub = (CPR >= 64) ? lane : lane % CPR;
-  float pre[VEC ? NIT * 4 : NIT];
-  const int64_t rows_ld = (abl & 4) ? 0 : rows;
-  auto issue = [&](int64_t tile) {
-    const int64_t r0 = tile * TM + wave * 32;
-#pragma unroll
-    for (int it = 0; it < NIT; ++it) {
-      const int64_t row = r0 + (it / IPR) * RPI + rsub;
-      const int c = csub + 64 * (it % IPR);
-      if (VEC) {
-        const bool ok = (c * 4 < K) && (row < rows_ld);
-        const float4* p = ok ? reinterpret_cast<const float4*>(X + row * ldx + c * 4) : zero4;
-        const float4 v = *p;
-        pre[4 * it] = v.x; pre[4 * it + 1] = v.y; pre[4 * it + 2] = v.z; pre[4 * it + 3] = v.w;
-      } else {
-        const bool ok = (c < K) && (row < rows_ld);
-        const float* p = ok ? X + row * ldx + c : reinterpret_cast<const float*>(zero4);
-        pre[it] = *p;
-      }
-    }
-  };
-  const float pa = (act && !silu) ? slope : 1.f;
-  auto commit = [&]() {
-    if (act && silu) {
-#pragma unroll
-      for (int q = 0; q < (VEC ? NIT * 4 : NIT); ++q) pre[q] = gcl::silu_f(pre[q]);
-    } else {
-#pragma unroll
-      for (int q = 0; q < (VEC ? NIT * 4 : NIT); ++q) pre[q] = pre[q] > 0.f ? pre[q] : pre[q] * pa;
-    }
-#pragma unroll
-    for (int it = 0; it < NIT; ++it) {
-      const int r = (it / IPR) * RPI + rsub;
-      const int c = csub + 64 * (it % IPR);
-      if (VEC) {
-        if (c * 4 < KE) {
-          float2* d = reinterpret_cast<float2*>(Xw + r * KP + c * 4);
-          d[0] = make_float2(pre[4 * it], pre[4 * it + 1]);
-          d[1] = make_float2(pre[4 * it + 2], pre[4 * it + 3]);
-        }
-      } else {
-        if (c < KE) Xw[r * KP + c] = pre[it];
-      }
-    }
-  };
-
-  float bj[NS];
-#pragma unroll
-  for (int s = 0; s < NS; ++s) {
-    const int j = s * 32 + (lane & 31);
-    bj[s] = (EPI == EPI_BIAS && bias && j < N) ? bias[j] : 0.f;
-  }
-  const bool has_z = (EPI == EPI_DX) && (Z != nullptr);
-
-  issue(blockIdx.x);
-  __syncthreads();
-  for (int64_t t = blockIdx.x; t < ntiles; t += gridDim.x) {
-    if (!gcl_lin_sync()) __builtin_amdgcn_fence(__ATOMIC_ACQ_REL, "wavefront");
-    else __syncthreads();
-    commit();
-    if (gcl_lin_sync()) __syncthreads();
-    issue(t + gridDim.x);
-
-    const int64_t r0 = t * TM;
-    const int64_t nr = (rows - r0) < TM ? (rows - r0) : TM;
-    const __amdgpu_buffer_rsrc_t ry = make_rsrc(Y + r0 * ldy, (abl & 1) ? 0 : win_bytes(nr, ldy, N));
-    const __amdgpu_buffer_rsrc_t rz = make_rsrc(has_z ? Z + r0 * ldz : Y, has_z ? win_bytes(nr, ldz, N) : 0);
-
-    f32x16 acc[NS];
-#pragma unroll
-    for (int s = 0; s < NS; ++s)
-#pragma unroll
-      for (int r = 0; r < 16; ++r) acc[s][r] = 0.f;
-
-    constexpr bool ZPRE = lin_zpre(NS, EPI);
-    float zpre[ZPRE ? NS : 1][16];
-    if (ZPRE) {
-#pragma unroll
-      for (int s = 0; s < NS; ++s) {
-        const int j = s * 32 + (lane & 31);
-#pragma unroll
-        for (int r = 0; r < 16; ++r) {
-          const int rr = wave * 32 + d_row(r, lane);
-          zpre[ZPRE ? s : 0][r] = buf_ld1(rz, (j < N) ? (unsigned)((rr * ldz + j) * 4) : kOOB);
-        }
-      }
-    }
-
-    const float* ap = Xw + (lane & 31) * KP + 2 * (lane >> 5);
-    const float* bp = Wl + (lane & 31) * KP + 2 * (lane >> 5);
-    const int nq = (abl & 2) ? 0 : (KE >> 2);
-    float2 a_c = *reinterpret_cast<const float2*>(ap);
-    float2 b_c[NS];
-#pragma unroll
-    for (int s = 0; s < NS; ++s) b_c[s] = *reinterpret_cast<const float2*>(bp + s * 32 * KP);
-    for (int q = 0; q < nq; ++q) {
-      const int qn = (q + 1 < nq) ? q + 1 : q;
-      const float2 a_n = *reinterpret_cast<const float2*>(ap + qn * 4);
-      float2 b_n[NS];
-#pragma unroll
-      for (int s = 0; s < NS; ++s) b_n[s] = *reinterpret_cast<const float2*>(bp + s * 32 * KP + qn * 4);
-#pragma unroll
-      for (int s = 0; s < NS; ++s) acc[s] = __builtin_amdgcn_mfma_f32_32x32x2f32(a_c.x, b_c[s].x, acc[s], 0, 0, 0);
-#pragma unroll
-      for (int s = 0; s < NS; ++s) acc[s] = __builtin_amdgcn_mfma_f32_32x32x2f32(a_c.y, b_c[s].y, acc[s], 0, 0, 0);
-      a_c = a_n;
-#pragma unroll
-      for (int s = 0; s < NS; ++s) b_c[s] = b_n[s];
-    }
-
-#pragma unroll
-    for (int s = 0; s < NS; ++s) {
-      const int j = s * 32 + (lane & 31);
-      const bool jok = j < N;
-      if (EPI == EPI_DX) {
-        float zv[16];
-#pragma unroll
-        for (int r = 0; r < 16; ++r) {
-          const int rr = wave * 32 + d_row(r, lane);
-          if (ZPRE) zv[r] = zpre[ZPRE ? s : 0][r];
-          else zv[r] = buf_ld1(rz, jok ? (unsigned)((rr * ldz + j) * 4) : kOOB);
-        }
-#pragma unroll
-        for (int r = 0; r < 16; ++r) {
-          const int rr = wave * 32 + d_row(r, lane);
-          float v = acc[s][r];
-          if (silu) {
-            v *= has_z ? gcl::dsilu_f(zv[r]) : 1.f;
-          } else {
-            const bool neg = has_z && !(zv[r] > 0.f);
-            slope_acc += neg ? (double)(v * zv[r]) : 0.0;
-            v = neg ? v * zs : v;
-          }
-          buf_st1<GCL_ST_AUX>(ry, jok ? (unsigned)((rr * ldy + j) * 4) : kOOB, v);
-        }
-      } else {
-#pragma unroll
-        for (int r = 0; r < 16; ++r) {
-          const int rr = wave * 32 + d_row(r, lane);
-          buf_st1<GCL_ST_AUX>(ry, jok ? (unsigned)((rr * ldy + j) * 4) : kOOB, acc[s][r] + bj[s]);
-        }
-      }
-    }
-  }
-
-  if (EPI == EPI_DX && slope_part) {
-    for (int off = 32; off > 0; off >>= 1) slope_acc += __shfl_down(slope_acc, off, 64);
-    __syncthreads();
-    double* dred = reinterpret_cast<double*>(smem);
-    if (lane == 0) dred[wave] = slope_acc;
-    __syncthreads();
-    if (tid == 0) {
-      double tot = 0.0;
-      for (int wv = 0; wv < (NT >> 6); ++wv) tot += dred[wv];
-      slope_part[blockIdx.x] = tot;
-    }
-  }
-}
+#define GCL_KERNEL_NAME linear_mfma_kernel
+#define GCL_SRC_PARTS false
+#define GCL_SRC_PARAM
+#define GCL_SRC_LOCAL const RowSrc src{};
+#include "linear_mfma_kernel.inc"
+#undef GCL_KERNEL_NAME
+#undef GCL_SRC_PARTS
+#undef GCL_SRC_PARAM
+#undef GCL_SRC_LOCAL
+#define GCL_KERNEL_NAME linear_mfma_parts_kernel
+#define GCL_SRC_PARTS true
+#define GCL_SRC_PARAM , RowSrc src
+#define GCL_SRC_LOCAL
+#include "linear_mfma_kernel.inc"
+#undef GCL_KERNEL_NAME
+#undef GCL_SRC_PARTS
+#undef GCL_SRC_PARAM
+#undef GCL_SRC_LOCAL
 
 template <int EPI>
 __global__ __launch_bounds__(256) void linear_valu_kernel(const float* __restrict__ X, int64_t ldx,
@@ -281,144 +167,24 @@
   static constexpr int min_waves = (PRE <= 8 && TO * TC <= 2) ? 3 : (PRE <= 16 && TO * TC <= 4) ? 2 : 1;
 };
 
-template <int NO, int NC, bool VEC>
-__global__ __launch_bounds__(256, (DwCfg<NO, NC>::min_waves)) void dw_mfma_kernel(
-    const float* __restrict__ dY, int64_t lddy, const float* __restrict__ X, int64_t ldx,
-    const float* __restrict__ in_slope, float* __restrict__ part, float* __restrict__ dbpart, int64_t rows,
-    int32_t Fin_all, int32_t Fout, int64_t rows_per_block, int32_t akind, int64_t tile_stride) {
-  using Cfg = DwCfg<NO, NC>;
-  const int ct = blockIdx.y;
-  X += (int64_t)ct * 128;
-  part += (int64_t)ct * tile_stride;
-  if (ct != 0) dbpart = nullptr;
-  const int Fin = (Fin_all - ct * 128) < 128 ? (Fin_all - ct * 128) : 128;
-  constexpr int WO = Cfg::WO, WC = Cfg::WC, TO = Cfg::TO, TC = Cfg::TC, PRE = Cfg::PRE;
-  constexpr int FoutP = Cfg::FoutP, FinP = Cfg::FinP;
-  extern __shared__ __align__(16) float smem[];
-  float* Yl = smem;
-  float* Xl = smem + (size_t)kDwRT * FoutP;
-  const int tid = threadIdx.x, lane = tid & 63, wave = tid >> 6;
-  const int li = lane & 31, lk = lane >> 5;
-  const int wo = wave % WO, wc = wave / WO;
-  const float slope = in_slope ? *in_slope : 1.f;
-  const bool act = akind != gcl::kActNone;
-  const int64_t rb = (int64_t)blockIdx.x * rows_per_block;
-  const int64_t re = min(rows, rb + rows_per_block);
-  const int nrows = (int)(re - rb);
-
-  f32x16 acc[TO][TC];
-#pragma unroll
-  for (int a = 0; a < TO; ++a)
-#pragma unroll
-    for (int c = 0; c < TC; ++c)
-#pragma unroll
-      for (int r = 0; r < 16; ++r) acc[a][c][r] = 0.f;
-  float dbacc[TO];
-#pragma unroll
-  for (int a = 0; a < TO; ++a) dbacc[a] = 0.f;
-
-  const int rs = tid >> 3, cg = tid & 7;
-  float4 pre[PRE];
-  const float* ybase = dY + rb * lddy;
-  const float* xbase = X + rb * ldx;
-  auto ld_slot = [&](const float* base, int rr, int c4, int64_t ld, int F) -> float4 {
-    const bool ok = rr < nrows;
-    const float* z = reinterpret_cast<const float*>(zero4);
-    const float* src = base + (int64_t)rr * ld + c4;
-    if (VEC) return *reinterpret_cast<const float4*>((ok && c4 < F) ? src : z);
-    float4 v;
-    v.x = *((ok && c4 < F) ? src : z);
-    v.y = *((ok && c4 + 1 < F) ? src + 1 : z);
-    v.z = *((ok && c4 + 2 < F) ? src + 2 : z);
-    v.w = *((ok && c4 + 3 < F) ? src + 3 : z);
-    return v;
-  };
-  auto issue = [&](int rel0) {
-#pragma unroll
-    for (int it = 0; it < PRE; ++it) {
-      const int j = it >> 1;
-      const int rr = rel0 + rs + 32 * (it & 1);
-      if (j < NO) pre[it] = ld_slot(ybase, rr, (cg + 8 * j) * 4, lddy, Fout);
-      else pre[it] = ld_slot(xbase, rr, (cg + 8 * (j - NO)) * 4, ldx, Fin);
-    }
-  };
-  auto commit = [&]() {
-#pragma unroll
-    for (int it = 0; it < PRE; ++it) {
-      const int j = it >> 1;
-      const int r = rs + 32 * (it & 1);
-      float4 v = pre[it];
-      if (j < NO) {
-        *reinterpret_cast<float4*>(Yl + r * FoutP + (cg + 8 * j) * 4) = v;
-      } else {
-        if (act) {
-          v.x = gcl::act_f(v.x, slope, akind); v.y = gcl::act_f(v.y, slope, akind);
-          v.z = gcl::act_f(v.z, slope, akind); v.w = gcl::act_f(v.w, slope, akind);
-        }
-        *reinterpret_cast<float4*>(Xl + r * FinP + (cg + 8 * (j - NO)) * 4) = v;
-      }
-    }
-  };
-
-  issue(0);
-  for (int rel0 = 0; rel0 < nrows; rel0 += kDwRT) {
-    __syncthreads();
-    commit();
-    __syncthreads();
-    issue(rel0 + kDwRT);
-    const float* yp = Yl + lk * FoutP + li;
-    const float* xp = Xl + lk * FinP + li;
-    float av[TO], bv[TC];
-#pragma unroll
-    for (int a = 0; a < TO; ++a) av[a] = yp[(wo + a * WO) * 32];
-#pragma unroll
-    for (int c = 0; c < TC; ++c) {
-      const int sc = wc + c * WC;
-      bv[c] = (sc < NC) ? xp[sc * 32] : 0.f;
-    }
-    for (int k = 0; k < kDwRT; k += 2) {
-      const int kn = (k + 2 < kDwRT) ? k + 2 : k;
-      float an[TO], bn[TC];
-#pragma unroll
-      for (int a = 0; a < TO; ++a) an[a] = yp[kn * FoutP + (wo + a * WO) * 32];
-#pragma unroll
-      for (int c = 0; c < TC; ++c) {
-        const int sc = wc + c * WC;
-        bn[c] = (sc < NC) ? xp[kn * FinP + sc * 32] : 0.f;
-      }
-#pragma unroll
-      for (int a = 0; a < TO; ++a) {
-        dbacc[a] += av[a];
-#pragma unroll
-        for (int c = 0; c < TC; ++c)
-          acc[a][c] = __builtin_amdgcn_mfma_f32_32x32x2f32(av[a], bv[c], acc[a][c], 0, 0, 0);
-      }
-#pragma unroll
-      for (int a = 0; a < TO; ++a) av[a] = an[a];
-#pragma unroll
-      for (int c = 0; c < TC; ++c) bv[c] = bn[c];
-    }
-  }
-
-  float* out = part + (size_t)blockIdx.x * FoutP * FinP;
-#pragma unroll
-  for (int a = 0; a < TO; ++a) {
-    const int so = wo + a * WO;
-#pragma unroll
-    for (int c = 0; c < TC; ++c) {
-      const int sc = wc + c * WC;
-      if (sc < NC) {
-#pragma unroll
-        for (int r = 0; r < 16; ++r)
-          out[(size_t)(so * 32 + d_row(r, lane)) * FinP + sc * 32 + li] = acc[a][c][r];
-      }
-    }
-    if (dbpart && wc == 0) {
-      const float d = dbacc[a] + __shfl_xor(dbacc[a], 32, 64);
-      if (lane < 32) dbpart[(size_t)blockIdx.x * FoutP + so * 32 + lane] = d;
-    }
-  }
-}
+#define GCL_KERNEL_NAME dw_mfma_kernel
+#define GCL_SRC_PARTS false
+#define GCL_SRC_PARAM
+#define GCL_SRC_LOCAL const RowSrc src{};
+#include "dw_mfma_kernel.inc"
+#undef GCL_KERNEL_NAME
+#undef GCL_SRC_PARTS
+#undef GCL_SRC_PARAM
+#undef GCL_SRC_LOCAL
+#define GCL_KERNEL_NAME dw_mfma_parts_kernel
+#define GCL_SRC_PARTS true
+#define GCL_SRC_PARAM , RowSrc src
+#define GCL_SRC_LOCAL
+#include "dw_mfma_kernel.inc"
+#undef GCL_KERNEL_NAME
+#undef GCL_SRC_PARTS
+#undef GCL_SRC_PARAM
+#undef GCL_SRC_LOCAL
 
 template <int NO, int NC>
 __global__ __launch_bounds__(256, 1) void linear_bwd_fused_kernel(
@@ -1298,9 +1064,22 @@
                           in_slope, d_in_slope, nullptr, 0, dx, lddx, rows, Fin, Fout, ws, ws_bytes, stream);
 }
 
+template <int NO, int NC, bool V>
+static int launch_dw_parts(const float* dy, int64_t lddy, const RowSrc& src, float* part, float* dbpart, int64_t rows,
+                           int32_t Fout, int64_t rpb, int64_t tile_stride, unsigned nblk, size_t lds, hipStream_t st) {
+  if constexpr (NC >= 3) {
+    auto kern = dw_mfma_parts_kernel<NO, NC, V>;
+    const int K = src.Cdyn + src.Cs;
+    GCL_ENSURE_DYN_LDS(kern, gcl::kLdsBytes);
+    hipLaunchKernelGGL(kern, dim3(nblk, 1u), dim3(256), lds, st, dy, lddy, (const float*)nullptr, (int64_t)K,
+                       (const float*)nullptr, part, dbpart, rows, K, Fout, rpb, (int32_t)gcl::kActNone, tile_stride, src);
+  }
+  return GCL_OK;
+}
+
 static int dw_block(const float* dy, int64_t lddy, const float* x, int64_t ldx, int akind, const float* in_slope,
                     float* dW, int64_t lddw, float* db, int64_t rows, int32_t Fin, int32_t Fout, int32_t accumulate,
-                    void* ws, hipStream_t st, gcl_reduce_job* job = nullptr) {
+                    void* ws, hipStream_t st, gcl_reduce_job* job = nullptr, const RowSrc* src = nullptr) {
   const int nct = (Fin + 127) / 128;
   const int NC = nct > 1 ? 4 : (Fin + 31) / 32;
   int NO = (Fout + 31) / 32;
@@ -1317,9 +1096,15 @@
   float* part = (float*)ws;
   float* dbpart = part + (size_t)kDwBlocks * FoutP * FinP;
   const int64_t tile_stride = (int64_t)nblk * FoutP * FinP;
-  const bool vec = (lddy % 4 == 0) && (ldx % 4 == 0) && gcl::aligned16(dy) && gcl::aligned16(x);
+  const bool vec = (lddy % 4 == 0) && gcl::aligned16(dy) && (src || ((ldx % 4 == 0) && gcl::aligned16(x)));
 #define GCL_DW3(NO_, NC_, V_)                                                                                     \
   do {                                                                                                            \
+    if (src) {                                                                                                    \
+      if (int rc_ = launch_dw_parts<NO_, NC_, V_>(dy, lddy, *src, part, db ? dbpart : nullptr, rows, Fout, rpb,   \
+                                                  tile_stride, (unsigned)nblk, lds, st))                          \
+        return rc_;                                                                                               \
+      break;                                                                                                      \
+    }                                                                                                             \
     auto kern = dw_mfma_kernel<NO_, NC_, V_>;                                                                     \
     GCL_ENSURE_DYN_LDS(kern, gcl::kLdsBytes);                                                                     \
     hipLaunchKernelGGL(kern, dim3((unsigned)nblk, (unsigned)nct), dim3(256), lds, st, dy, lddy, x, ldx, in_slope, part, \
@@ -1397,10 +1182,10 @@
 static int dense_bwd_dw_impl(const float* dy, int64_t lddy, const float* x, int64_t ldx, int32_t act,
                              const float* slope, float* dW, int64_t lddw, float* db, int64_t rows, int32_t Fin,
                              int32_t Fout, int32_t accumulate, void* ws, size_t ws_bytes, gcl_stream_t stream,
-                             gcl_reduce_job* job) {
+                             gcl_reduce_job* job, const RowSrc* src = nullptr) {
   if (job) memset(job, 0, 2 * sizeof(*job));
   if (Fout > 256) job = nullptr;
-  GCL_CHECK_ARG(dy && x && dW, "dense_bwd_dw: null argument");
+  GCL_CHECK_ARG(dy && (x || src) && dW, "dense_bwd_dw: null argument");
   GCL_CHECK_ARG(lddy >= Fout && ldx >= Fin && lddw >= Fin, "dense_bwd_dw: leading dimension too small");
   GCL_CHECK_ARG(Fin >= 1 && Fout >= 1, "dense_bwd_dw: bad shape");
   GCL_CHECK_ARG(lddw < (1 << 30), "dense_bwd_dw: lddw too large");
@@ -1410,7 +1195,7 @@
   for (int o0 = 0; o0 < Fout; o0 += 256) {
     const int fo = Fout - o0 < 256 ? Fout - o0 : 256;
     int rc = dw_block(dy + o0, lddy, x, ldx, act, sl, dW + (int64_t)o0 * lddw, lddw, db ? db + o0 : nullptr, rows, Fin,
-                      fo, accumulate, ws, (hipStream_t)stream, job);
+                      fo, accumulate, ws, (hipStream_t)stream, job, src);
     if (rc) return rc;
   }
   return GCL_OK;
@@ -1446,6 +1231,80 @@
                                  void* ws, size_t ws_bytes, gcl_stream_t stream) {
   return gcl_dense_bwd_dw(dy, lddy, x, ldx, in_slope ? GCL_ACT_PRELU : GCL_ACT_NONE, in_slope, dW, Fin, db, rows, Fin,
                           Fout, accumulate, ws, ws_bytes, stream);
+}
+
+static bool aligned8(const void* p) { return (reinterpret_cast<uintptr_t>(p) & 7) == 0; }
+
+extern "C" int gcl_input_parts_ok(const gcl_input_parts* p, int32_t Fout) {
+  if (!p || gcl::env_int("GCL_NO_INPUT_PARTS", 0) == 1) return 0;
+  if (p->B < 1 || p->G < 1 || p->M < 0 || p->r < 0 || p->r > p->M || p->Cdyn < 2 || p->Cs < 2) return 0;
+  if ((p->Cdyn & 1) || (p->Cs & 1)) return 0;
+  const int K = p->Cdyn + p->Cs;
+  if (K < 65 || K > 128 || Fout < 1 || Fout > 256) return 0;
+  if (!p->x || !p->grid_static || p->ldx != p->Cdyn) return 0;
+  if ((p->r < p->M && !p->mesh_static) || (p->r > 0 && (!p->tail || p->tail_width != K))) return 0;
+  if (!aligned8(p->x) || !aligned8(p->grid_static) || !aligned8(p->mesh_static) || !aligned8(p->tail)) return 0;
+  if (p->G + (int64_t)p->M < 2 || (int64_t)p->B * (p->G + (int64_t)p->M) * K >= ((int64_t)1 << 31)) return 0;
+  if (use_valu() || !panel_fits(K, Fout, K % 4 == 0, false, true)) return 0;
+  return 1;
+}
+
+static RowSrc row_src(const gcl_input_parts* p) {
+  return RowSrc{p->x, p->grid_static, p->mesh_static, p->tail, p->G, p->G + p->M, p->Cdyn, p->Cs, p->r};
+}
+
+extern "C" int gcl_dense_fwd_parts(const gcl_input_parts* p, const float* W, const float* bias, float* y, int64_t ldy,
+                                   int32_t Fout, gcl_stream_t stream) {
+  GCL_CHECK_ARG(p && W && y && ldy >= Fout, "dense_fwd_parts: null argument or ldy < Fout");
+  GCL_CHECK_ARG(gcl_input_parts_ok(p, Fout), "dense_fwd_parts: input refused (gcl_input_parts_ok)");
+  const int K = p->Cdyn + p->Cs;
+  const int64_t rows = (int64_t)p->B * (p->G + p->M);
+  LinGeom g;
+  if (int rc = lin_geom(rows, K, Fout, true, &g)) return rc;
+  const RowSrc src = row_src(p);
+  const size_t lds = ((size_t)g.NS * 32 + 32 * g.waves) * (((K + 3) & ~3) + 2) * sizeof(float) + g.waves * 96 * sizeof(float*);
+  GCL_CHECK_ARG(lds <= gcl::kLdsBytes, "dense_fwd_parts: K=%d Fout=%d needs %zu B of LDS", K, Fout, lds);
+#define GCL_LINP(NS_)                                                                                             \
+  do {                                                                                                            \
+    auto kern = linear_mfma_parts_kernel<NS_, EPI_BIAS, 128, true>;                                               \
+    GCL_ENSURE_DYN_LDS(kern, gcl::kLdsBytes);                                                                     \
+    hipLaunchKernelGGL(kern, dim3(g.grid), dim3(g.waves * 64), lds, (hipStream_t)stream, (const float*)nullptr,   \
+                       (int64_t)K, (const float*)nullptr, W, K, 0, bias, y, ldy, rows, K, Fout,                   \
+                       (const float*)nullptr, (int64_t)0, (const float*)nullptr, (double*)nullptr,                \
+                       (int32_t)gcl::kActNone, gcl_ablate(), src);                                                \
+  } while (0)
+  switch (g.NS) {
+    case 1: GCL_LINP(1); break;
+    case 2: GCL_LINP(2); break;
+    case 4: GCL_LINP(4); break;
+    default: GCL_LINP(8); break;
+  }
+#undef GCL_LINP
+  GCL_CHECK_LAUNCH();
+  return GCL_OK;
+}
+
+static int dw_parts_impl(const float* dy, int64_t lddy, const gcl_input_parts* p, float* dW, int64_t lddw, float* db,
+                         int32_t Fout, int32_t accumulate, void* ws, size_t ws_bytes, gcl_stream_t stream,
+                         gcl_reduce_job* job) {
+  GCL_CHECK_ARG(p && gcl_input_parts_ok(p, Fout), "dense_bwd_dw_parts: input refused (gcl_input_parts_ok)");
+  const RowSrc src = row_src(p);
+  const int K = p->Cdyn + p->Cs;
+  return dense_bwd_dw_impl(dy, lddy, nullptr, K, GCL_ACT_NONE, nullptr, dW, lddw, db, (int64_t)p->B * (p->G + p->M), K,
+                           Fout, accumulate, ws, ws_bytes, stream, job, &src);
+}
+
+extern "C" int gcl_dense_bwd_dw_parts(const float* dy, int64_t lddy, const gcl_input_parts* p, float* dW, int64_t lddw,
+                                      float* db, int32_t Fout, int32_t accumulate, void* ws, size_t ws_bytes,
+                                      gcl_stream_t stream) {
+  return dw_parts_impl(dy, lddy, p, dW, lddw, db, Fout, accumulate, ws, ws_bytes, stream, nullptr);
+}
+
+extern "C" int gcl_dense_bwd_dw_parts_deferred(const float* dy, int64_t lddy, const gcl_input_parts* p, float* dW,
+                                               int64_t lddw, float* db, int32_t Fout, int32_t accumulate, void* ws,
+                                               size_t ws_bytes, gcl_stream_t stream, gcl_reduce_job* job) {
+  GCL_CHECK_ARG(job, "dense_bwd_dw_parts_deferred: null job");
+  return dw_parts_impl(dy, lddy, p, dW, lddw, db, Fout, accumulate, ws, ws_bytes, stream, job);
 }
 
 static bool fused_ok(const float* dy, int64_t lddy, const float* x, int64_t ldx, const float* dx, int64_t lddx,
diff --git a/graphcast-lite_amd/csrc/linear_mfma_kernel.inc b/graphcast-lite_amd/csrc/linear_mfma_kernel.inc
--- /dev/null
+++ b/graphcast-lite_amd/csrc/linear_mfma_kernel.inc
@@ -0,0 +1,245 @@
+template <int NS, int EPI, int KT, bool VEC>
+__global__ __launch_bounds__(256, lin_min_waves(NS, KT)) void GCL_KERNEL_NAME(const float* __restrict__ X, int64_t ldx,
+                                                          const float* __restrict__ in_slope,
+                                                          const float* __restrict__ W, int32_t ldw, int32_t trans,
+                                                          const float* __restrict__ bias, float* __restrict__ Y,
+                                                          int64_t ldy, int64_t rows, int32_t K, int32_t N,
+                                                          const float* __restrict__ Z, int64_t ldz,
+                                                          const float* __restrict__ z_slope,
+                                                          double* __restrict__ slope_part, int32_t akind,
+                                                          int32_t abl GCL_SRC_PARAM) {
+  constexpr bool PARTS = GCL_SRC_PARTS;
+  GCL_SRC_LOCAL
+  static_assert(!PARTS || (VEC && KT == 128 && EPI == EPI_BIAS), "the row source feeds the 65..128-wide forward");
+  extern __shared__ __align__(16) float smem[];
+  const int KE = (K + 3) & ~3;
+  const int KP = KE + 2;
+  float* Wl = smem;
+  float* Xl = smem + (size_t)NS * 32 * KP;
+  const int tid = threadIdx.x, lane = tid & 63, wave = tid >> 6;
+  const int NT = blockDim.x;
+  const int TM = (NT >> 6) * 32;
+
+  for (int base = 0; base < NS * 32 * KE; base += NT * 8) {
+    float wv[8];
+#pragma unroll
+    for (int u = 0; u < 8; ++u) {
+      const int idx = base + u * NT + tid;
+      const int j = idx / KE, k = idx - j * KE;
+      const bool ok = (idx < NS * 32 * KE) && (j < N) && (k < K);
+      const float* src = ok ? (trans ? W + (int64_t)k * ldw + j : W + (int64_t)j * ldw + k)
+                            : reinterpret_cast<const float*>(zero4);
+      wv[u] = *src;
+    }
+#pragma unroll
+    for (int u = 0; u < 8; ++u) {
+      const int idx = base + u * NT + tid;
+      const int j = idx / KE, k = idx - j * KE;
+      if (idx < NS * 32 * KE) Wl[j * KP + k] = wv[u];
+    }
+  }
+  const float slope = in_slope ? *in_slope : 1.f;
+  const bool act = EPI == EPI_BIAS && akind != gcl::kActNone;
+  const bool silu = akind == gcl::kActSilu;
+  float* Xw = Xl + (size_t)wave * 32 * KP;
+  const int64_t ntiles = (rows + TM - 1) / TM;
+  double slope_acc = 0.0;
+  const float zs = (EPI == EPI_DX && z_slope) ? *z_slope : 1.f;
+
+  constexpr int CPR = VEC ? KT / 4 : KT;
+  constexpr int RPI = CPR >= 64 ? 1 : 64 / CPR;
+  constexpr int IPR = CPR >= 64 ? CPR / 64 : 1;
+  constexpr int NIT = (32 / RPI) * IPR;
+  const int rsub = (CPR >= 64) ? 0 : lane / CPR;
+  const int csub = (CPR >= 64) ? lane : lane % CPR;
+  float pre[VEC ? NIT * 4 : NIT];
+  const int64_t rows_ld = (abl & 4) ? 0 : rows;
+  const float** ptab = reinterpret_cast<const float**>(Xl + (size_t)(NT >> 6) * 32 * KP) + wave * 96;
+  int pe[2] = {0, 0}, po[2] = {0, 0};
+  if constexpr (PARTS) {
+#pragma unroll
+    for (int h = 0; h < 2; ++h) {
+      const int c = csub * 4 + 2 * h;
+      pe[h] = c >= K ? 2 : c < src.Cdyn ? 0 : 1;
+      po[h] = c >= K ? 0 : c < src.Cdyn ? c : c - src.Cdyn;
+    }
+  }
+  RowRef nx;
+  auto locate = [&](int64_t tile) {
+    if constexpr (PARTS) {
+      const uint32_t row = (uint32_t)(tile * TM + wave * 32 + (lane & 31));
+      const uint32_t b = row / (uint32_t)src.GM;
+      nx = src.row(b, row - b * (uint32_t)src.GM, (int64_t)row < rows_ld);
+    }
+  };
+  auto issue = [&](int64_t tile) {
+    const int64_t r0 = tile * TM + wave * 32;
+    if constexpr (PARTS) {
+      static_assert(!PARTS || (IPR == 1 && RPI == 2), "two rows per wave-instruction");
+      const float** trow = ptab + (lane & 31) * 3;
+      trow[0] = nx.dyn; trow[1] = nx.st; trow[2] = zero_row;
+      __builtin_amdgcn_fence(__ATOMIC_ACQ_REL, "wavefront");
+#pragma unroll
+      for (int it = 0; it < NIT; ++it) {
+        const float2 lo = ldg2(ptab[(2 * it + rsub) * 3 + pe[0]] + po[0]);
+        const float2 hi = ldg2(ptab[(2 * it + rsub) * 3 + pe[1]] + po[1]);
+        pre[4 * it] = lo.x; pre[4 * it + 1] = lo.y; pre[4 * it + 2] = hi.x; pre[4 * it + 3] = hi.y;
+      }
+      return;
+    }
+#pragma unroll
+    for (int it = 0; it < NIT; ++it) {
+      const int64_t row = r0 + (it / IPR) * RPI + rsub;
+      const int c = csub + 64 * (it % IPR);
+      if (VEC) {
+        const bool ok = (c * 4 < K) && (row < rows_ld);
+        const float4* p = ok ? reinterpret_cast<const float4*>(X + row * ldx + c * 4) : zero4;
+        const float4 v = *p;
+        pre[4 * it] = v.x; pre[4 * it + 1] = v.y; pre[4 * it + 2] = v.z; pre[4 * it + 3] = v.w;
+      } else {
+        const bool ok = (c < K) && (row < rows_ld);
+        const float* p = ok ? X + row * ldx + c : reinterpret_cast<const float*>(zero4);
+        pre[it] = *p;
+      }
+    }
+  };
+  const float pa = (act && !silu) ? slope : 1.f;
+  auto commit = [&]() {
+    if (act && silu) {
+#pragma unroll
+      for (int q = 0; q < (VEC ? NIT * 4 : NIT); ++q) pre[q] = gcl::silu_f(pre[q]);
+    } else {
+#pragma unroll
+      for (int q = 0; q < (VEC ? NIT * 4 : NIT); ++q) pre[q] = pre[q] > 0.f ? pre[q] : pre[q] * pa;
+    }
+#pragma unroll
+    for (int it = 0; it < NIT; ++it) {
+      const int r = (it / IPR) * RPI + rsub;
+      const int c = csub + 64 * (it % IPR);
+      if (VEC) {
+        if (c * 4 < KE) {
+          float2* d = reinterpret_cast<float2*>(Xw + r * KP + c * 4);
+          d[0] = make_float2(pre[4 * it], pre[4 * it + 1]);
+          d[1] = make_float2(pre[4 * it + 2], pre[4 * it + 3]);
+        }
+      } else {
+        if (c < KE) Xw[r * KP + c] = pre[it];
+      }
+    }
+  };
+
+  float bj[NS];
+#pragma unroll
+  for (int s = 0; s < NS; ++s) {
+    const int j = s * 32 + (lane & 31);
+    bj[s] = (EPI == EPI_BIAS && bias && j < N) ? bias[j] : 0.f;
+  }
+  const bool has_z = (EPI == EPI_DX) && (Z != nullptr);
+
+  locate(blockIdx.x);
+  issue(blockIdx.x);
+  locate((int64_t)blockIdx.x + gridDim.x);
+  __syncthreads();
+  for (int64_t t = blockIdx.x; t < ntiles; t += gridDim.x) {
+    if (!gcl_lin_sync()) __builtin_amdgcn_fence(__ATOMIC_ACQ_REL, "wavefront");
+    else __syncthreads();
+    commit();
+    if (gcl_lin_sync()) __syncthreads();
+    issue(t + gridDim.x);
+    locate(t + 2 * (int64_t)gridDim.x);
+
+    const int64_t r0 = t * TM;
+    const int64_t nr = (rows - r0) < TM ? (rows - r0) : TM;
+    const __amdgpu_buffer_rsrc_t ry = make_rsrc(Y + r0 * ldy, (abl & 1) ? 0 : win_bytes(nr, ldy, N));
+    const __amdgpu_buffer_rsrc_t rz = make_rsrc(has_z ? Z + r0 * ldz : Y, has_z ? win_bytes(nr, ldz, N) : 0);
+
+    f32x16 acc[NS];
+#pragma unroll
+    for (int s = 0; s < NS; ++s)
+#pragma unroll
+      for (int r = 0; r < 16; ++r) acc[s][r] = 0.f;
+
+    constexpr bool ZPRE = lin_zpre(NS, EPI);
+    float zpre[ZPRE ? NS : 1][16];
+    if (ZPRE) {
+#pragma unroll
+      for (int s = 0; s < NS; ++s) {
+        const int j = s * 32 + (lane & 31);
+#pragma unroll
+        for (int r = 0; r < 16; ++r) {
+          const int rr = wave * 32 + d_row(r, lane);
+          zpre[ZPRE ? s : 0][r] = buf_ld1(rz, (j < N) ? (unsigned)((rr * ldz + j) * 4) : kOOB);
+        }
+      }
+    }
+
+    const float* ap = Xw + (lane & 31) * KP + 2 * (lane >> 5);
+    const float* bp = Wl + (lane & 31) * KP + 2 * (lane >> 5);
+    const int nq = (abl & 2) ? 0 : (KE >> 2);
+    float2 a_c = *reinterpret_cast<const float2*>(ap);
+    float2 b_c[NS];
+#pragma unroll
+    for (int s = 0; s < NS; ++s) b_c[s] = *reinterpret_cast<const float2*>(bp + s * 32 * KP);
+    for (int q = 0; q < nq; ++q) {
+      const int qn = (q + 1 < nq) ? q + 1 : q;
+      const float2 a_n = *reinterpret_cast<const float2*>(ap + qn * 4);
+      float2 b_n[NS];
+#pragma unroll
+      for (int s = 0; s < NS; ++s) b_n[s] = *reinterpret_cast<const float2*>(bp + s * 32 * KP + qn * 4);
+#pragma unroll
+      for (int s = 0; s < NS; ++s) acc[s] = __builtin_amdgcn_mfma_f32_32x32x2f32(a_c.x, b_c[s].x, acc[s], 0, 0, 0);
+#pragma unroll
+      for (int s = 0; s < NS; ++s) acc[s] = __builtin_amdgcn_mfma_f32_32x32x2f32(a_c.y, b_c[s].y, acc[s], 0, 0, 0);
+      a_c = a_n;
+#pragma unroll
+      for (int s = 0; s < NS; ++s) b_c[s] = b_n[s];
+    }
+
+#pragma unroll
+    for (int s = 0; s < NS; ++s) {
+      const int j = s * 32 + (lane & 31);
+      const bool jok = j < N;
+      if (EPI == EPI_DX) {
+        float zv[16];
+#pragma unroll
+        for (int r = 0; r < 16; ++r) {
+          const int rr = wave * 32 + d_row(r, lane);
+          if (ZPRE) zv[r] = zpre[ZPRE ? s : 0][r];
+          else zv[r] = buf_ld1(rz, jok ? (unsigned)((rr * ldz + j) * 4) : kOOB);
+        }
+#pragma unroll
+        for (int r = 0; r < 16; ++r) {
+          const int rr = wave * 32 + d_row(r, lane);
+          float v = acc[s][r];
+          if (silu) {
+            v *= has_z ? gcl::dsilu_f(zv[r]) : 1.f;
+          } else {
+            const bool neg = has_z && !(zv[r] > 0.f);
+            slope_acc += neg ? (double)(v * zv[r]) : 0.0;
+            v = neg ? v * zs : v;
+          }
+          buf_st1<GCL_ST_AUX>(ry, jok ? (unsigned)((rr * ldy + j) * 4) : kOOB, v);
+        }
+      } else {
+#pragma unroll
+        for (int r = 0; r < 16; ++r) {
+          const int rr = wave * 32 + d_row(r, lane);
+          buf_st1<GCL_ST_AUX>(ry, jok ? (unsigned)((rr * ldy + j) * 4) : kOOB, acc[s][r] + bj[s]);
+        }
+      }
+    }
+  }
+
+  if (EPI == EPI_DX && slope_part) {
+    for (int off = 32; off > 0; off >>= 1) slope_acc += __shfl_down(slope_acc, off, 64);
+    __syncthreads();
+    double* dred = reinterpret_cast<double*>(smem);
+    if (lane == 0) dred[wave] = slope_acc;
+    __syncthreads();
+    if (tid == 0) {
+      double tot = 0.0;
+      for (int wv = 0; wv < (NT >> 6); ++wv) tot += dred[wv];
+      slope_part[blockIdx.x] = tot;
+    }
+  }
+}
diff --git a/graphcast-lite_amd/functional.py b/graphcast-lite_amd/functional.py
--- a/graphcast-lite_amd/functional.py
+++ b/graphcast-lite_amd/functional.py
@@ -84,12 +84,13 @@
     def forward(ctx, x, owner, has_ln: bool, eps: float, *params):
         L = (len(params) - (2 if has_ln else 0) + 1) // 3
         shape = x.shape
-        x2 = hip.rows2d(x.detach())
+        parts = x if isinstance(x, hip.InputParts) else None
+        x2 = parts if parts is not None else hip.rows2d(x.detach())
         zs = []
         cur, slope = x2, None
         out = stats = None
         for k in range(L):
-            if 2 <= L - k <= 3:
+            if 2 <= L - k <= 3 and cur is not parts:
                 tail = hip.mlp_fwd_chain(cur, [params[3 * j].detach() for j in range(k, L)],
                                          [params[3 * j + 1].detach() for j in range(k, L)],
                                          [params[3 * j + 2].detach() for j in range(k, L - 1)], slope,
@@ -99,7 +100,10 @@
                     cur, out, stats = tail[0][-1], tail[1], tail[2]
                     break
             W, b = params[3 * k], params[3 * k + 1]
-            z = hip.linear_fwd(cur, W.detach(), b.detach(), slope)
+            if cur is parts:
+                z = hip.linear_fwd_parts(parts, W.detach(), b.detach())
+            else:
+                z = hip.linear_fwd(cur, W.detach(), b.detach(), slope)
             zs.append(z)
             cur = z
             slope = params[3 * k + 2].detach() if k < L - 1 else None
@@ -127,6 +131,10 @@
         else:
             dz = dy2
         dx = None
+        if isinstance(ctx.x2, hip.InputParts):
+            dw_of = hip.linear_bwd_dw_parts
+        else:
+            dw_of = lambda dz_, x_, dW_, db_, acc_: hip.linear_bwd_dw(dz_, x_, None, dW_, db_, acc_)
         for k in range(L - 1, -1, -1):
             W = params[3 * k].detach()
             inp = ctx.x2 if k == 0 else zs[k - 1]
@@ -140,10 +148,10 @@
                 dx = hip.linear_bwd_all(dz, W, inp, None, None, dW, db, None, G.acc[wi], acc_db=G.acc[bi],
                                         act=hip.ACT_NONE)
             elif db is not None and G.acc[bi] != G.acc[wi]:
-                hip.linear_bwd_dw(dz, inp, None, dW, None, G.acc[wi])
+                dw_of(dz, inp, dW, None, G.acc[wi])
                 hip.colsum(dz, db, G.acc[bi])
             else:
-                hip.linear_bwd_dw(dz, inp, None, dW, db, G.acc[wi])
+                dw_of(dz, inp, dW, db, G.acc[wi])
         if dx is not None:
             dx = dx.view(dy.shape[:-1] + (dx.shape[-1],))
         return (dx, None, None, None) + G.out()
diff --git a/graphcast-lite_amd/hip.py b/graphcast-lite_amd/hip.py
--- a/graphcast-lite_amd/hip.py
+++ b/graphcast-lite_amd/hip.py
@@ -83,6 +83,10 @@
     "gcl_colsum_split": (C.c_int, [_vp, _i64, _i64, _vp, _i64, _i64, _i32, _i32, _i32, _i32, _vp, _i32, _vp, _sz, _vp]),
     "gcl_assemble_input": (C.c_int, [_vp, _vp, _vp, _vp, _i64, _i32, _i32, _i32, _i32, _i32, _vp]),
     "gcl_assemble_input_tail": (C.c_int, [_vp, _vp, _vp, _vp, _i32, _vp, _i64, _i32, _i32, _i32, _i32, _i32, _vp]),
+    "gcl_input_parts_ok": (C.c_int, [_vp, _i32]),
+    "gcl_dense_fwd_parts": (C.c_int, [_vp, _vp, _vp, _vp, _i64, _i32, _vp]),
+    "gcl_dense_bwd_dw_parts": (C.c_int, [_vp, _i64, _vp, _vp, _i64, _vp, _i32, _i32, _vp, _sz, _vp]),
+    "gcl_dense_bwd_dw_parts_deferred": (C.c_int, [_vp, _i64, _vp, _vp, _i64, _vp, _i32, _i32, _vp, _sz, _vp, _vp]),
     "gcl_wmse_fwd_bwd": (C.c_int, [_vp, _i64, _i64, _vp, _i64, _i64, _vp, _i64, _i64, _vp, _vp, _f32, _f32, _vp,
                                    _vp, _vp, _vp, _i32, _i32, _i32, _vp, _sz, _vp]),
     "gcl_wmse_fwd_bwd_ld": (C.c_int, [_vp, _i64, _i64, _vp, _i64, _i64, _vp, _i64, _i64, _vp, _vp, _f32, _f32, _vp, _i64, _i64,
@@ -897,6 +901,76 @@
     return out
 
 
+class _InputPartsC(C.Structure):
+    _fields_ = [("x", _vp), ("grid_static", _vp), ("mesh_static", _vp), ("tail", _vp), ("ldx", _i64), ("B", _i32),
+                ("G", _i32), ("M", _i32), ("Cdyn", _i32), ("Cs", _i32), ("r", _i32), ("tail_width", _i32)]
+
+
+class InputParts:
+
+    def __init__(self, tensors, c, shape):
+        self.tensors, self.c, self.shape = tensors, c, shape
+        self.device = tensors[0].device
+
+    @property
+    def rows(self):
+        return self.shape[0] * self.shape[1]
+
+
+def _parts_struct(x3, grid_static, mesh_static, tail3):
+    B, G, Cdyn = x3.shape
+    Cs = grid_static.shape[1]
+    r = tail3.shape[1] if tail3 is not None else 0
+    M = mesh_static.shape[0] if mesh_static is not None else r
+    ptr = lambda t: t.data_ptr() if t is not None else None
+    return _InputPartsC(ptr(x3), ptr(grid_static), ptr(mesh_static), ptr(tail3), x3.stride(1), B, G, M, Cdyn, Cs, r,
+                        tail3.shape[2] if tail3 is not None else 0)
+
+
+def input_parts(x3, grid_static, mesh_static, tail3, W):
+    ts = [t for t in (x3, grid_static, mesh_static, tail3, W) if t is not None]
+    if x3.dim() != 3 or grid_static.dim() != 2 or W.dim() != 2 or (mesh_static is None and tail3 is None):
+        return None
+    if any(t.dtype != torch.float32 or not t.is_contiguous() or t.device != x3.device for t in ts):
+        return None
+    B, G, Cdyn = x3.shape
+    Cs = grid_static.shape[1]
+    if grid_static.shape[0] != G or W.shape[1] != Cdyn + Cs or B * G == 0:
+        return None
+    if mesh_static is not None and (mesh_static.dim() != 2 or mesh_static.shape[1] != Cs):
+        return None
+    if tail3 is not None and (tail3.dim() != 3 or tail3.shape[0] != B):
+        return None
+    c = _parts_struct(x3, grid_static, mesh_static, tail3)
+    if not lib().gcl_input_parts_ok(C.addressof(c), W.shape[0]):
+        return None
+    return InputParts(ts[:-1], c, (B, G + c.M, Cdyn + Cs))
+
+
+def linear_fwd_parts(parts: InputParts, W, bias):
+    Fout = W.shape[0]
+    _p(parts.tensors[0])
+    out = torch.empty(parts.rows, Fout, dtype=torch.float32, device=parts.device)
+    _check(lib().gcl_dense_fwd_parts(C.addressof(parts.c), _p(W), _p(bias), _p(out), Fout, Fout, _stream()))
+    return out
+
+
+def linear_bwd_dw_parts(dy, parts: InputParts, dW, db, accumulate: bool):
+    rows, Fout = dy.shape
+    Fin = parts.shape[2]
+    assert rows == parts.rows and tuple(dW.shape) == (Fout, Fin) and dW.stride(1) == 1
+    _p(parts.tensors[0])
+    nb = lib().gcl_linear_bwd_ws_bytes(rows, Fin, Fout)
+    if _deferred.active:
+        _queue(nb, dy.device, (dW, db), 2, lambda ws, jobs: lib().gcl_dense_bwd_dw_parts_deferred(
+            _p(dy), _ld(dy), C.addressof(parts.c), _p(dW), dW.stride(0), _p(db), Fout, 1 if accumulate else 0,
+            ws.data_ptr(), ws.numel(), _stream(), C.cast(jobs, C.c_void_p)))
+        return
+    ws = workspace(nb, dy.device)
+    _check(lib().gcl_dense_bwd_dw_parts(_p(dy), _ld(dy), C.addressof(parts.c), _p(dW), dW.stride(0), _p(db), Fout,
+                                        1 if accumulate else 0, ws.data_ptr(), ws.numel(), _stream()))
+
+
 def wmse_fwd_bwd(delta3, x_last3, y3, node_w, chan_w, inv_wsum, grad_scale, want_grad=True, want_state=False,
                  loss_prev=None, ldd_out=None):
     B, G, Cc = delta3.shape
diff --git a/graphcast-lite_amd/models.py b/graphcast-lite_amd/models.py
--- a/graphcast-lite_amd/models.py
+++ b/graphcast-lite_amd/models.py
@@ -698,12 +698,12 @@
                     if lat_pre is not None:
                         land.want_split_out()
             if self._mlp_on_folded_rows and self.encoder.mlp is not None and f.rd > 0:
-                x_m = AssembleFn.apply(X3, self.init_grid_features, f.mstat2, f.x_tail2)
+                x_m = self._encoder_input(X3, f.mstat2, f.x_tail2)
                 h_m = self.encoder.mlp(X=x_m)
                 x_g = MeshLatFn.apply(h_m, f.maps_e, f.ne, G + f.r, f.rd, None)
                 enc_c = self.encoder.graph_layer(X=x_g, edge_index=c.enc_graph, **ekw)
             else:
-                x_c = AssembleFn.apply(X3, self.init_grid_features, f.mstat, f.x_fold if f.r > 0 else None)
+                x_c = self._encoder_input(X3, f.mstat, f.x_fold if f.r > 0 else None)
                 enc_c = self.encoder.forward(X=x_c, edge_index=c.enc_graph, **ekw)
             tail = land.split_tail() if land is not None else None
             if tail is not None:
@@ -749,6 +749,14 @@
             return out[0], grid_lat[0], processed[0]
         return out, grid_lat, processed
 
+    def _encoder_input(self, X3, mesh_static, tail3):
+        mlp = self.encoder.mlp
+        if mlp is not None and not X3.requires_grad and isinstance(mlp.MLP[0], nn.Linear):
+            parts = hip.input_parts(X3, self.init_grid_features, mesh_static, tail3, mlp.MLP[0].weight)
+            if parts is not None:
+                return parts
+        return AssembleFn.apply(X3, self.init_grid_features, mesh_static, tail3)
+
     _lat_through_table = os.environ.get("GCL_NO_LAT_TABLE", "0") in ("0", "")
     _mlp_on_folded_rows = os.environ.get("GCL_NO_MLP_FOLD", "0") in ("0", "")
     _ln_into_decoder_input = os.environ.get("GCL_NO_LN_MAP", "0") in ("0", "")
diff --git a/include/gcl.h b/include/gcl.h
--- a/include/gcl.h
+++ b/include/gcl.h
@@ -222,6 +222,24 @@
                             int32_t r, float* out, int64_t ldo, int32_t B, int32_t G, int32_t M, int32_t Cdyn,
                             int32_t Cs, gcl_stream_t stream);
 
+typedef struct gcl_input_parts {
+  const float* x;
+  const float* grid_static;
+  const float* mesh_static;
+  const float* tail;
+  int64_t ldx;
+  int32_t B, G, M, Cdyn, Cs, r;
+  int32_t tail_width;
+} gcl_input_parts;
+int gcl_input_parts_ok(const gcl_input_parts* parts, int32_t Fout);
+int gcl_dense_fwd_parts(const gcl_input_parts* parts, const float* W, const float* bias, float* y, int64_t ldy,
+                        int32_t Fout, gcl_stream_t stream);
+int gcl_dense_bwd_dw_parts(const float* dy, int64_t lddy, const gcl_input_parts* parts, float* dW, int64_t lddw,
+                           float* db, int32_t Fout, int32_t accumulate, void* ws, size_t ws_bytes, gcl_stream_t stream);
+int gcl_dense_bwd_dw_parts_deferred(const float* dy, int64_t lddy, const gcl_input_parts* parts, float* dW,
+                                    int64_t lddw, float* db, int32_t Fout, int32_t accumulate, void* ws,
+                                    size_t ws_bytes, gcl_stream_t stream, gcl_reduce_job* job );
+
 int gcl_wmse_fwd_bwd(const float* delta, int64_t ldd, int64_t bsd, const float* x_last, int64_t ldx,
                      int64_t bsx, const float* y, int64_t ldy_, int64_t bsy, const float* node_w,
                      const float* chan_w, float inv_wsum, float grad_scale, float* d_delta,
```

After: 28490 (median of 6 runs). No clear change (+0.6%).
